# sergivalverde/sub-cortical_segmentation

Hardware: NVIDIA B200
Metric: voxels_per_sec_full_volume_inference (higher is better)
Workload: dtype bf16

## Files before the change

sub-cortical_segmentation_b200/csrc/conv_sweep.cu:

```cuda
#include "tc_common.cuh"

namespace sc {

constexpr int SW_SLOT_HALF = 17408;
constexpr int SW_MAX_SLOTS = 14;
constexpr int SW_BAR_BYTES = 512;

struct SweepArgs {
  int Pw, R;
  int bn;
  int S;
  int nstrips, strip_w;
  int nseg, L;
  int n_items;
  int stages;
  int out_bufs;
  int npanels;
  int in_dx, in_dy;
  const float* scale; const float* shift; const float* alpha;
  unsigned long long* dbg;
  const uint8_t* item_on;
  double* stats;
  int st_H, st_pitch;
};

__device__ __forceinline__ void sweep_mma(uint32_t acc, uint32_t a_lo, uint32_t b_lo, uint32_t idesc, uint32_t accumulate, uint32_t elected) {
  asm volatile(
      "{\n\t"
      ".reg .pred p, q;\n\t"
      ".reg .b64 da, db;\n\t"
      "setp.ne.b32 p, %4, 0;\n\t"
      "setp.ne.b32 q, %5, 0;\n\t"
      "mov.b64 da, {%1, %6};\n\t"
      "mov.b64 db, {%2, %6};\n\t"
      "@q tcgen05.mma.cta_group::1.kind::f16 [%0], da, db, %3, p;\n\t"
      "}" ::"r"(acc), "r"(a_lo), "r"(b_lo), "r"(idesc), "r"(accumulate), "r"(elected), "r"(0x40004040u) : "memory");
}
__device__ __forceinline__ uint32_t desc_lo(uint32_t saddr) { return ((saddr & 0x3FFFFu) >> 4) | (1u << 16); }

__device__ __forceinline__ void tmem_ld16(uint32_t taddr, uint32_t (&r)[16]) {
  asm volatile(
      "tcgen05.ld.sync.aligned.32x32b.x16.b32 {%0, %1, %2, %3, %4, %5, %6, %7, %8, %9, %10, %11, %12, %13, %14, %15}, [%16];"
      : "=r"(r[0]), "=r"(r[1]), "=r"(r[2]), "=r"(r[3]), "=r"(r[4]), "=r"(r[5]), "=r"(r[6]), "=r"(r[7]), "=r"(r[8]),
        "=r"(r[9]), "=r"(r[10]), "=r"(r[11]), "=r"(r[12]), "=r"(r[13]), "=r"(r[14]), "=r"(r[15])
      : "r"(taddr));
}

__device__ __forceinline__ void tmem_ld8(uint32_t taddr, uint32_t (&r)[8]) {
  asm volatile("tcgen05.ld.sync.aligned.32x32b.x8.b32 {%0, %1, %2, %3, %4, %5, %6, %7}, [%8];"
               : "=r"(r[0]), "=r"(r[1]), "=r"(r[2]), "=r"(r[3]), "=r"(r[4]), "=r"(r[5]), "=r"(r[6]), "=r"(r[7])
               : "r"(taddr));
}
template <int CW>
__device__ __forceinline__ void sweep_stats_flush(float (&st_s)[CW], float (&st_q)[CW], float* s_red , int ew, int c0,
                                                  bool real, int lane, double* stats) {
#pragma unroll
  for (int k = 0; k < CW; ++k)
#pragma unroll
    for (int o = 16; o; o >>= 1) { st_s[k] += __shfl_xor_sync(0xffffffffu, st_s[k], o); st_q[k] += __shfl_xor_sync(0xffffffffu, st_q[k], o); }
  if (lane == 0) {
#pragma unroll
    for (int k = 0; k < CW; ++k) { s_red[ew * 2 * CW + k] = st_s[k]; s_red[ew * 2 * CW + CW + k] = st_q[k]; }
  }
  asm volatile("bar.sync 7, 512;" ::: "memory");
  if ((ew & 3) == 0 && real && lane < 2 * CW) {
    const int base = ew * 2 * CW + lane;
    const float tot = s_red[base] + s_red[base + 2 * CW] + s_red[base + 4 * CW] + s_red[base + 6 * CW];
    const int mom = lane / CW, ch = c0 + (lane - mom * CW);
    if (ch < 64) atomicAdd(&stats[ch * 2 + mom], (double)tot);
  }
}

template <int CW>
__device__ __forceinline__ void tmem_ld(uint32_t taddr, uint32_t (&r)[CW]) {
  if constexpr (CW == 16) tmem_ld16(taddr, r); else tmem_ld8(taddr, r);
}
template <int CW>
__device__ __forceinline__ void tmem_zero(uint32_t taddr) {
  if constexpr (CW == 16)
    asm volatile("tcgen05.st.sync.aligned.32x32b.x16.b32 [%0], {%1, %1, %1, %1, %1, %1, %1, %1, %1, %1, %1, %1, %1, %1, %1, %1};"
                 ::"r"(taddr), "r"(0u) : "memory");
  else
    asm volatile("tcgen05.st.sync.aligned.32x32b.x8.b32 [%0], {%1, %1, %1, %1, %1, %1, %1, %1};" ::"r"(taddr), "r"(0u) : "memory");
}
template <int CW>
__device__ __forceinline__ void sweep_acc_clear(uint32_t tcol, int S, int bn) {
  for (int j = 0; j < S + 2; ++j) tmem_zero<CW>(tcol + (uint32_t)(j * bn));
  asm volatile("tcgen05.wait::st.sync.aligned;" ::: "memory");
}
template <int CW, bool PAIR>
__device__ __forceinline__ void sweep_drain(uint64_t* afull, uint64_t* aempty, uint32_t& dj, uint32_t& dph, int S, int bn,
                                            uint32_t tcol, bool real, bool keep, int lane, float (&acc)[CW], bool timed,
                                            uint32_t& w_wait) {
  const long long c0 = timed ? clock64() : 0;
  mbar_wait(&afull[dj], (dph >> dj) & 1u);
  dph ^= 1u << dj;
  if (timed) w_wait += (uint32_t)(clock64() - c0);
  asm volatile("tcgen05.fence::after_thread_sync;" ::: "memory");
  if (real) {
    const uint32_t taddr = tcol + dj * (uint32_t)bn, tspill = taddr + (uint32_t)(S * bn);
    const bool split = dj < 2;
    if (keep) {
#pragma unroll
      for (int h = 0; h < CW; h += 8) {
        uint32_t r1[8], r2[8];
        tmem_ld8(taddr + h, r1);
        if (split) tmem_ld8(tspill + h, r2);
        asm volatile("tcgen05.wait::ld.sync.aligned;" ::: "memory");
#pragma unroll
        for (int k = 0; k < 8; ++k) acc[h + k] = split ? __uint_as_float(r1[k]) + __uint_as_float(r2[k]) : __uint_as_float(r1[k]);
      }
    }
    tmem_zero<CW>(taddr);
    if (split) tmem_zero<CW>(tspill);
    asm volatile("tcgen05.wait::st.sync.aligned;" ::: "memory");
  }
  asm volatile("tcgen05.fence::before_thread_sync;" ::: "memory");
  __syncwarp();
  if (lane == 0) {
    if (PAIR) mbar_arrive_cta(&aempty[dj], 0); else mbar_arrive(&aempty[dj]);
  }
  if (++dj == (uint32_t)S) dj = 0;
}
__device__ __forceinline__ void sweep_claim(uint64_t* aempty, uint32_t j, uint32_t& eph) {
  mbar_wait(&aempty[j], ((eph >> j) & 1u) ^ 1u);
  eph ^= 1u << j;
}
__device__ __forceinline__ uint32_t slot_back(uint32_t j, uint32_t k, int S) { return j >= k ? j - k : j + (uint32_t)S - k; }
__device__ __forceinline__ void tma_store_3d(const CUtensorMap* map, const void* src, int c0, int c1, int c2) {
  asm volatile("cp.async.bulk.tensor.3d.global.shared::cta.bulk_group [%0, {%2, %3, %4}], [%1];"
               ::"l"(reinterpret_cast<uint64_t>(map)), "r"(smem_u32(src)), "r"(c0), "r"(c1), "r"(c2) : "memory");
}
template <int KSTEPS, int DIL, int POOL, int CW, bool LO64, bool OUT32>
__global__ void __launch_bounds__(576, 1)
conv_sweep_kernel(const __grid_constant__ CUtensorMap mapA, const __grid_constant__ CUtensorMap mapW, const __grid_constant__ CUtensorMap mapO,
                  const SweepArgs a) {
  extern __shared__ uint8_t smem_raw[];
  uint8_t* smem = smem_raw + ((1024u - (smem_u32(smem_raw) & 1023u)) & 1023u);
  constexpr int BOXPX = 128 + 2 * DIL;
  constexpr int BOX_BYTES = BOXPX * 128;
  constexpr int NBOX = LO64 ? 1 : 2;
  constexpr int SLOT = NBOX * SW_SLOT_HALF;
  constexpr int LO_OFF = LO64 ? 64 : SW_SLOT_HALF;
  const int half_bytes = 3 * a.bn * 128;
  const int panel_bytes = 2 * half_bytes;
  const int w_bytes = a.npanels * panel_bytes;
  uint8_t* sW = smem;
  uint8_t* sRing = smem + w_bytes;
  constexpr int OB_BYTES = OUT32 ? 16384 : 32768;
  uint8_t* sOut = sRing + a.stages * SLOT;
  uint64_t* bars = reinterpret_cast<uint64_t*>(sOut + a.out_bufs * OB_BYTES);
  uint64_t* full = bars;
  uint64_t* empty = bars + a.stages;
  uint64_t* afull = bars + 2 * a.stages;
  uint64_t* aempty = afull + a.S;
  uint64_t* wfull = aempty + a.S;
  uint32_t* tmem_slot = reinterpret_cast<uint32_t*>(wfull + 1);
  float* s_const = reinterpret_cast<float*>(tmem_slot + 2);
  float* s_xch = s_const + 192;

  const int warp = threadIdx.x >> 5, lane = threadIdx.x & 31;

  if (threadIdx.x == 0) {
    for (int s = 0; s < a.stages; ++s) { mbar_init(&full[s], 1); mbar_init(&empty[s], 1); }
    for (int j = 0; j < a.S; ++j) { mbar_init(&afull[j], 1); mbar_init(&aempty[j], 16); }
    mbar_init(wfull, 1);
    asm volatile("fence.mbarrier_init.release.cluster;" ::: "memory");
  }
  if (warp == 1) {
    asm volatile("tcgen05.alloc.cta_group::1.sync.aligned.shared::cta.b32 [%0], %1;" ::"r"(smem_u32(tmem_slot)), "r"(512) : "memory");
    asm volatile("tcgen05.relinquish_alloc_permit.cta_group::1.sync.aligned;" ::: "memory");
  }
  for (int i = threadIdx.x; i < 64; i += blockDim.x) {
    const bool ok = i < a.bn;
    s_const[i] = ok ? __ldg(a.scale + i) : 0.f;
    s_const[64 + i] = ok ? __ldg(a.shift + i) : 0.f;
    s_const[128 + i] = ok ? __ldg(a.alpha + i) : 0.f;
  }
  for (int i = threadIdx.x; i < a.out_bufs * OB_BYTES / 16; i += blockDim.x)
    reinterpret_cast<uint4*>(sOut)[i] = make_uint4(0u, 0u, 0u, 0u);
  asm volatile("fence.proxy.async.shared::cta;" ::: "memory");
  asm volatile("tcgen05.fence::before_thread_sync;" ::: "memory");
  __syncthreads();
  asm volatile("tcgen05.fence::after_thread_sync;" ::: "memory");
  const uint32_t tmem_base = *tmem_slot;
  const int q4 = warp & 3, ew = warp - 2, grp = ew >> 2, c0 = grp * CW;
  const bool real = c0 < a.bn;
  const uint32_t tcol = tmem_base + ((uint32_t)(q4 * 32) << 16) + (uint32_t)c0;
  if (warp >= 2 && real) sweep_acc_clear<CW>(tcol, a.S, a.bn);
  asm volatile("tcgen05.fence::before_thread_sync;" ::: "memory");
  __syncthreads();
  asm volatile("tcgen05.fence::after_thread_sync;" ::: "memory");

  auto decode = [&](int item, int& w0, int& q, int& n0, int& Lc) {
    const int strip = item % a.nstrips;
    const int rest = item / a.nstrips;
    q = rest % DIL;
    const int seg = rest / DIL;
    w0 = strip * a.strip_w;
    const int Nq = (a.R - q + DIL - 1) / DIL;
    n0 = seg * a.L;
    Lc = Nq - n0 < a.L ? Nq - n0 : a.L;
  };

  if (warp == 0) {
    if (lane == 0) {
      asm volatile("prefetch.tensormap [%0];" ::"l"(reinterpret_cast<uint64_t>(&mapA)) : "memory");
      asm volatile("prefetch.tensormap [%0];" ::"l"(reinterpret_cast<uint64_t>(&mapW)) : "memory");
      asm volatile("prefetch.tensormap [%0];" ::"l"(reinterpret_cast<uint64_t>(&mapO)) : "memory");
      mbar_expect_tx(wfull, (uint32_t)w_bytes);
      for (int p = 0; p < 2 * a.npanels; ++p) tma_load_2d(&mapW, wfull, sW + p * half_bytes, 0, p * 3 * a.bn);
      uint32_t g = 0;
      long long w_empty = 0;
      const long long tstart = a.dbg ? clock64() : 0;
      for (int item = blockIdx.x; item < a.n_items; item += gridDim.x) {
        int w0, q, n0, Lc;
        decode(item, w0, q, n0, Lc);
        if (Lc <= 0 || (a.item_on && !a.item_on[item])) continue;
        const int nload = Lc + (POOL == 1 ? 1 : 0) + 2;
        for (int m = 0; m < nload; ++m, ++g) {
          const uint32_t s = g % a.stages, use = g / a.stages;
          if (use > 0) {
            const long long c0 = a.dbg ? clock64() : 0;
            mbar_wait(&empty[s], (use - 1) & 1);
            if (a.dbg) w_empty += clock64() - c0;
          }
          mbar_expect_tx(&full[s], (uint32_t)(NBOX * BOX_BYTES));
          uint8_t* sp = sRing + s * SLOT;
          const int r = q + DIL * (n0 + m);
          tma_load_3d(&mapA, &full[s], sp, 0, w0 + a.in_dx, r + a.in_dy);
          if (NBOX == 2) tma_load_3d(&mapA, &full[s], sp + SW_SLOT_HALF, 64, w0 + a.in_dx, r + a.in_dy);
        }
      }
      if (a.dbg) { a.dbg[blockIdx.x * 8 + 0] = (unsigned long long)w_empty; a.dbg[blockIdx.x * 8 + 1] = (unsigned long long)(clock64() - tstart); }
    }
    __syncwarp();
  } else if (warp == 1) {
    const uint32_t leader = elect_one();
    const uint32_t idesc = (1u << 4) | (1u << 7) | (1u << 10) | ((uint32_t)(3 * a.bn >> 3) << 17) | ((uint32_t)(128 >> 4) << 24);
    mbar_wait(wfull, 0);
    const uint32_t w_lo = desc_lo(smem_u32(sW));
    const uint32_t ring_lo = desc_lo(smem_u32(sRing));
    const uint32_t panel16 = (uint32_t)(panel_bytes >> 4), wl_off = (uint32_t)(half_bytes >> 4);
    uint32_t rs = 0, rph = 0;
    uint32_t j = 2, eph = 0;
    bool open = false;
    long long w_full = 0, w_tempty = 0;
    const long long tstart = a.dbg ? clock64() : 0;
    for (int item = blockIdx.x; item < a.n_items; item += gridDim.x) {
      int w0, q, n0, Lc;
      decode(item, w0, q, n0, Lc);
      if (Lc <= 0 || (a.item_on && !a.item_on[item])) continue;
      const int nin = Lc + (POOL == 1 ? 1 : 0) + 2;
      const uint32_t j0 = (uint32_t)(n0 + 2) % (uint32_t)a.S;
      const uint32_t d = open ? (j0 + (uint32_t)a.S - j) % (uint32_t)a.S : 2u;
      if (d) {
        if (open && leader) { umma_commit(&afull[slot_back(j, 2, a.S)]); if (d >= 2) umma_commit(&afull[slot_back(j, 1, a.S)]); }
        if (d >= 2) sweep_claim(aempty, slot_back(j0, 2, a.S), eph);
        sweep_claim(aempty, slot_back(j0, 1, a.S), eph);
      }
      j = j0; open = true;
      for (int m = 0; m < nin; ++m) {
        long long c0 = a.dbg ? clock64() : 0;
        sweep_claim(aempty, j, eph);
        if (a.dbg) { const long long c1 = clock64(); w_tempty += c1 - c0; c0 = c1; }
        mbar_wait(&full[rs], rph);
        if (a.dbg) w_full += clock64() - c0;
        asm volatile("tcgen05.fence::after_thread_sync;" ::: "memory");
        const uint32_t p = slot_back(j, 2, a.S);
        const uint32_t acc = tmem_base + p * (uint32_t)a.bn;
        const uint32_t sl = ring_lo + rs * (SLOT >> 4);
#pragma unroll
        for (int kx = 0; kx < 3; ++kx) {
#pragma unroll
          for (int ks = 0; ks < KSTEPS; ++ks) {
            const int gk = kx * KSTEPS + ks;
            const uint32_t a_hi = sl + (uint32_t)(kx * DIL * 8 + ks * 2);
            const uint32_t a_lo = a_hi + (uint32_t)(LO_OFF >> 4);
            const uint32_t wh = w_lo + (uint32_t)(gk >> 2) * panel16 + (uint32_t)((gk & 3) * 2);
            sweep_mma(acc, a_lo, wh, idesc, 1, leader);
            sweep_mma(acc, a_hi, wh + wl_off, idesc, 1, leader);
            sweep_mma(acc, a_hi, wh, idesc, 1, leader);
          }
        }
        if (leader) {
          umma_commit(&empty[rs]);
          umma_commit(&afull[p]);
        }
        __syncwarp();
        if (++rs == (uint32_t)a.stages) { rs = 0; rph ^= 1; }
        if (++j == (uint32_t)a.S) j = 0;
      }
    }
    if (open && leader) {
      umma_commit(&afull[slot_back(j, 2, a.S)]);
      umma_commit(&afull[slot_back(j, 1, a.S)]);
    }
    __syncwarp();
    if (a.dbg && leader) {
      a.dbg[blockIdx.x * 8 + 2] = (unsigned long long)w_full; a.dbg[blockIdx.x * 8 + 3] = (unsigned long long)w_tempty;
      a.dbg[blockIdx.x * 8 + 4] = (unsigned long long)(clock64() - tstart);
    }
  } else {
    const int px = q4 * 32 + lane;
    const bool issuer = threadIdx.x == 64;
    const int trow = POOL == 2 ? px >> 1 : px;
    const bool writer = POOL == 2 ? !(lane & 1) : true;
    const uint32_t row_off = (uint32_t)trow * 128u;
    const uint32_t sw = (uint32_t)(trow & 7);
    const uint32_t hi_chunk = (uint32_t)(c0 >> 3);
    const uint32_t lo_base = OUT32 ? 0u : 16384u, lo_chunk = OUT32 ? 4u + hi_chunk : hi_chunk;
    uint32_t t = 0, e = 0;
    uint32_t dj = 0, dph = 0;
    uint32_t w_tfull = 0;
    const bool timed = a.dbg != nullptr;
    const long long tstart = a.dbg ? clock64() : 0;
    constexpr bool STATS = POOL == 0 && DIL == 1;
    float st_s[STATS ? CW : 1], st_q[STATS ? CW : 1];
#pragma unroll
    for (int k = 0; k < (STATS ? CW : 1); ++k) st_s[k] = st_q[k] = 0.f;
    float v[CW];
    for (int item = blockIdx.x; item < a.n_items; item += gridDim.x) {
      int w0, q, n0, Lc;
      decode(item, w0, q, n0, Lc);
      if (Lc <= 0 || (a.item_on && !a.item_on[item])) continue;
      const int nrow = Lc + (POOL == 1 ? 1 : 0);
      const uint32_t j0 = (uint32_t)(n0 + 2) % (uint32_t)a.S;
      const uint32_t d = (j0 + 2u * (uint32_t)a.S - 2u - dj) % (uint32_t)a.S;
      if (t == 0 || d >= 3) {
        if (t > 0)
          for (int h = 0; h < 2; ++h) sweep_drain<CW, false>(afull, aempty, dj, dph, a.S, a.bn, tcol, real, false, lane, v, timed, w_tfull);
        dj = slot_back(j0, 2, a.S);
      } else {
        for (uint32_t h = 0; h < d; ++h) sweep_drain<CW, false>(afull, aempty, dj, dph, a.S, a.bn, tcol, real, false, lane, v, timed, w_tfull);
      }
      for (int h = 0; h < 2; ++h) sweep_drain<CW, false>(afull, aempty, dj, dph, a.S, a.bn, tcol, real, false, lane, v, timed, w_tfull);
      float hprev[CW];
#pragma unroll
      for (int k = 0; k < CW; ++k) hprev[k] = 0.f;
      for (int m = 0; m < nrow; ++m, ++t) {
        sweep_drain<CW, false>(afull, aempty, dj, dph, a.S, a.bn, tcol, real, true, lane, v, timed, w_tfull);
        if (real) {
#pragma unroll
          for (int k4 = 0; k4 < CW / 4; ++k4) {
            const float4 sc_ = *reinterpret_cast<const float4*>(s_const + c0 + 4 * k4);
            const float4 sh = *reinterpret_cast<const float4*>(s_const + 64 + c0 + 4 * k4);
            const float4 al = *reinterpret_cast<const float4*>(s_const + 128 + c0 + 4 * k4);
            v[4 * k4 + 0] = prelu(fmaf(v[4 * k4 + 0], sc_.x, sh.x), al.x);
            v[4 * k4 + 1] = prelu(fmaf(v[4 * k4 + 1], sc_.y, sh.y), al.y);
            v[4 * k4 + 2] = prelu(fmaf(v[4 * k4 + 2], sc_.z, sh.z), al.z);
            v[4 * k4 + 3] = prelu(fmaf(v[4 * k4 + 3], sc_.w, sh.w), al.w);
          }
        }

        int r_out = q + DIL * (n0 + m);
        if (POOL == 1) {
          if (real) {
            float* xw = s_xch + (((t & 1) * 4 + grp) * 4 + q4) * 32;
            if (lane < DIL) {
#pragma unroll
              for (int k4 = 0; k4 < CW / 4; ++k4)
                *reinterpret_cast<float4*>(xw + lane * 16 + 4 * k4) = make_float4(v[4 * k4], v[4 * k4 + 1], v[4 * k4 + 2], v[4 * k4 + 3]);
            }
            asm volatile("bar.sync %0, 128;" ::"r"(1 + grp) : "memory");
            const bool edge = lane >= 32 - DIL;
            const float* xr = s_xch + (((t & 1) * 4 + grp) * 4 + ((q4 + 1) & 3)) * 32 + (edge ? (lane - (32 - DIL)) * 16 : 0);
#pragma unroll
            for (int k4 = 0; k4 < CW / 4; ++k4) {
              const float4 x4 = *reinterpret_cast<const float4*>(xr + 4 * k4);
              const float xs[4] = {x4.x, x4.y, x4.z, x4.w};
#pragma unroll
              for (int k = 0; k < 4; ++k) {
                float nb = __shfl_down_sync(0xffffffffu, v[4 * k4 + k], DIL);
                if (edge) nb = xs[k];
                const float h = fmaxf(v[4 * k4 + k], nb);
                v[4 * k4 + k] = fmaxf(h, hprev[4 * k4 + k]);
                hprev[4 * k4 + k] = h;
              }
            }
          }
          if (m == 0) continue;
          r_out -= DIL;
        }
        if (POOL == 2) {
          if (real) {
#pragma unroll
            for (int k = 0; k < CW; ++k) {
              const float h = fmaxf(v[k], __shfl_down_sync(0xffffffffu, v[k], 1));
              v[k] = fmaxf(h, hprev[k]);
              hprev[k] = (m & 1) ? 0.f : h;
            }
          }
          if (!(m & 1)) continue;
          r_out >>= 1;
        }
        if constexpr (STATS) {
          if (a.stats && real) {
            const int wpx = w0 + px;
            if (wpx < a.Pw && (wpx & (a.st_pitch - 1)) < a.st_H && r_out < a.st_H) {
#pragma unroll
              for (int k = 0; k < CW; ++k) { st_s[k] += v[k]; st_q[k] = fmaf(v[k], v[k], st_q[k]); }
            }
          }
        }
        uint8_t* ob = sOut + (e % (uint32_t)a.out_bufs) * OB_BYTES;
        if (a.out_bufs == 1) {
          if (issuer) asm volatile("cp.async.bulk.wait_group.read 0;" ::: "memory");
          asm volatile("bar.sync 5, 512;" ::: "memory");
        }
        if (real) {
          uint32_t hi[CW / 2], lo[CW / 2];
#pragma unroll
          for (int k = 0; k < CW / 2; ++k) split2(v[2 * k], v[2 * k + 1], hi[k], lo[k]);
#pragma unroll
          for (int c = 0; c < CW / 8; ++c) {
            if (!writer) break;
            *reinterpret_cast<uint4*>(ob + row_off + (((hi_chunk + c) ^ sw) << 4)) = make_uint4(hi[4 * c], hi[4 * c + 1], hi[4 * c + 2], hi[4 * c + 3]);
            *reinterpret_cast<uint4*>(ob + lo_base + row_off + (((lo_chunk + c) ^ sw) << 4)) = make_uint4(lo[4 * c], lo[4 * c + 1], lo[4 * c + 2], lo[4 * c + 3]);
          }
          asm volatile("fence.proxy.async.shared::cta;" ::: "memory");
        }
        if (a.out_bufs == 2 && issuer) asm volatile("cp.async.bulk.wait_group.read 0;" ::: "memory");
        asm volatile("bar.sync 6, 512;" ::: "memory");
        if (issuer) {
          tma_store_3d(&mapO, ob, 0, POOL == 2 ? w0 >> 1 : w0, r_out);
          if (!OUT32) tma_store_3d(&mapO, ob + 16384, 64, POOL == 2 ? w0 >> 1 : w0, r_out);
          asm volatile("cp.async.bulk.commit_group;" ::: "memory");
        }
        ++e;
      }
    }
    if (t > 0)
      for (int h = 0; h < 2; ++h) sweep_drain<CW, false>(afull, aempty, dj, dph, a.S, a.bn, tcol, real, false, lane, v, timed, w_tfull);
    if (issuer) asm volatile("cp.async.bulk.wait_group 0;" ::: "memory");
    if constexpr (STATS) {
      if (a.stats) sweep_stats_flush<CW>(st_s, st_q, s_xch, ew, c0, real, lane, a.stats);
    }
    if (a.dbg && threadIdx.x == 64) {
      a.dbg[blockIdx.x * 8 + 5] = (unsigned long long)w_tfull; a.dbg[blockIdx.x * 8 + 6] = (unsigned long long)(clock64() - tstart);
      a.dbg[blockIdx.x * 8 + 7] = t;
    }
  }
  asm volatile("tcgen05.fence::before_thread_sync;" ::: "memory");
  __syncthreads();
  if (warp == 1) {
    asm volatile("tcgen05.fence::after_thread_sync;" ::: "memory");
    asm volatile("tcgen05.dealloc.cta_group::1.sync.aligned.b32 %0, %1;" ::"r"(tmem_base), "r"(512) : "memory");
  }
}

__device__ __forceinline__ void sweep_mma_2sm(uint32_t acc, uint32_t a_lo, uint32_t b_lo, uint32_t idesc, uint32_t accumulate, uint32_t elected) {
  asm volatile(
      "{\n\t"
      ".reg .pred p, q;\n\t"
      ".reg .b64 da, db;\n\t"
      "setp.ne.b32 p, %4, 0;\n\t"
      "setp.ne.b32 q, %5, 0;\n\t"
      "mov.b64 da, {%1, %6};\n\t"
      "mov.b64 db, {%2, %6};\n\t"
      "@q tcgen05.mma.cta_group::2.kind::f16 [%0], da, db, %3, p;\n\t"
      "}" ::"r"(acc), "r"(a_lo), "r"(b_lo), "r"(idesc), "r"(accumulate), "r"(elected), "r"(0x40004040u) : "memory");
}

template <int KSTEPS, int DIL, int POOL>
__global__ void __cluster_dims__(2, 1, 1) __launch_bounds__(576, 1)
conv_sweep_pair_kernel(const __grid_constant__ CUtensorMap mapA, const __grid_constant__ CUtensorMap mapW, const __grid_constant__ CUtensorMap mapO,
                       const SweepArgs a) {
  extern __shared__ uint8_t smem_raw[];
  uint8_t* smem = smem_raw + ((1024u - (smem_u32(smem_raw) & 1023u)) & 1023u);
  constexpr int BOXPX = 128 + 2 * DIL;
  constexpr int BOX_BYTES = BOXPX * 128;
  constexpr int SLOT = 2 * SW_SLOT_HALF;
  constexpr int CW = 16;
  const int panel_bytes = 3 * a.bn * 128;
  const int w_bytes = a.npanels * panel_bytes;
  uint8_t* sW = smem;
  uint8_t* sRing = smem + ((w_bytes + 1023) & ~1023);
  constexpr int OB_BYTES = 32768;
  uint8_t* sOut = sRing + a.stages * SLOT;
  uint64_t* bars = reinterpret_cast<uint64_t*>(sOut + a.out_bufs * OB_BYTES);
  uint64_t* full = bars;
  uint64_t* empty = bars + a.stages;
  uint64_t* afull = bars + 2 * a.stages;
  uint64_t* aempty = afull + a.S;
  uint64_t* wfull = aempty + a.S;
  uint32_t* tmem_slot = reinterpret_cast<uint32_t*>(wfull + 1);
  float* s_const = reinterpret_cast<float*>(tmem_slot + 2);
  float* s_xch = s_const + 192;

  const int warp = threadIdx.x >> 5, lane = threadIdx.x & 31;
  const uint32_t rank = cluster_ctarank();
  const int pair = blockIdx.x >> 1, npairs = gridDim.x >> 1;

  if (threadIdx.x == 0) {
    for (int s = 0; s < a.stages; ++s) { mbar_init(&full[s], 1); mbar_init(&empty[s], 1); }
    for (int j = 0; j < a.S; ++j) { mbar_init(&afull[j], 1); mbar_init(&aempty[j], 32); }
    mbar_init(wfull, 1);
    asm volatile("fence.mbarrier_init.release.cluster;" ::: "memory");
  }
  if (warp == 1) {
    asm volatile("tcgen05.alloc.cta_group::2.sync.aligned.shared::cta.b32 [%0], %1;" ::"r"(smem_u32(tmem_slot)), "r"(512) : "memory");
    asm volatile("tcgen05.relinquish_alloc_permit.cta_group::2.sync.aligned;" ::: "memory");
  }
  for (int i = threadIdx.x; i < 64; i += blockDim.x) {
    const bool ok = i < a.bn;
    s_const[i] = ok ? __ldg(a.scale + i) : 0.f;
    s_const[64 + i] = ok ? __ldg(a.shift + i) : 0.f;
    s_const[128 + i] = ok ? __ldg(a.alpha + i) : 0.f;
  }
  for (int i = threadIdx.x; i < a.out_bufs * OB_BYTES / 16; i += blockDim.x)
    reinterpret_cast<uint4*>(sOut)[i] = make_uint4(0u, 0u, 0u, 0u);
  asm volatile("fence.proxy.async.shared::cta;" ::: "memory");
  asm volatile("tcgen05.fence::before_thread_sync;" ::: "memory");
  __syncthreads();
  asm volatile("tcgen05.fence::after_thread_sync;" ::: "memory");
  const uint32_t tmem_base = *tmem_slot;
  const int q4 = warp & 3, ew = warp - 2, grp = ew >> 2, c0 = grp * CW;
  const bool real = c0 < a.bn;
  const uint32_t tcol = tmem_base + ((uint32_t)(q4 * 32) << 16) + (uint32_t)c0;
  if (warp >= 2 && real) sweep_acc_clear<CW>(tcol, a.S, a.bn);
  asm volatile("tcgen05.fence::before_thread_sync;" ::: "memory");
  __syncthreads();
  cluster_sync_all();
  asm volatile("tcgen05.fence::after_thread_sync;" ::: "memory");

  const int nsp = (a.nstrips + 1) >> 1;
  auto decode = [&](int item, int& w0, int& q, int& n0, int& Lc) {
    const int sp = item % nsp;
    const int rest = item / nsp;
    q = rest % DIL;
    const int seg = rest / DIL;
    w0 = (2 * sp + (int)rank) * a.strip_w;
    const int Nq = (a.R - q + DIL - 1) / DIL;
    n0 = seg * a.L;
    Lc = Nq - n0 < a.L ? Nq - n0 : a.L;
  };

  if (warp == 0) {
    if (lane == 0) {
      asm volatile("prefetch.tensormap [%0];" ::"l"(reinterpret_cast<uint64_t>(&mapA)) : "memory");
      asm volatile("prefetch.tensormap [%0];" ::"l"(reinterpret_cast<uint64_t>(&mapW)) : "memory");
      asm volatile("prefetch.tensormap [%0];" ::"l"(reinterpret_cast<uint64_t>(&mapO)) : "memory");
      {
        const uint32_t lbar = smem_u32(wfull) & 0xFEFFFFFFu;
        if (rank == 0) mbar_expect_tx(wfull, (uint32_t)(2 * w_bytes));
        for (int p = 0; p < a.npanels; ++p) tma_load_2d_2sm(&mapW, lbar, sW + p * panel_bytes, 0, (p * 2 + (int)rank) * 3 * a.bn);
      }
      uint32_t g = 0;
      long long w_empty = 0;
      const long long tstart = a.dbg ? clock64() : 0;
      for (int item = pair; item < a.n_items; item += npairs) {
        int w0, q, n0, Lc;
        decode(item, w0, q, n0, Lc);
        if (Lc <= 0 || (a.item_on && !a.item_on[item])) continue;
        const int nload = Lc + (POOL == 1 ? 1 : 0) + 2;
        for (int m = 0; m < nload; ++m, ++g) {
          const uint32_t s = g % a.stages, use = g / a.stages;
          if (use > 0) {
            const long long c0w = a.dbg ? clock64() : 0;
            mbar_wait(&empty[s], (use - 1) & 1);
            if (a.dbg) w_empty += clock64() - c0w;
          }
          const uint32_t lbar = smem_u32(&full[s]) & 0xFEFFFFFFu;
          if (rank == 0) mbar_expect_tx(&full[s], (uint32_t)(2 * 2 * BOX_BYTES));
          uint8_t* sp = sRing + s * SLOT;
          const int r = q + DIL * (n0 + m);
          tma_load_3d_2sm(&mapA, lbar, sp, 0, w0 + a.in_dx, r + a.in_dy);
          tma_load_3d_2sm(&mapA, lbar, sp + SW_SLOT_HALF, 64, w0 + a.in_dx, r + a.in_dy);
        }
      }
      if (a.dbg) { a.dbg[blockIdx.x * 8 + 0] = (unsigned long long)w_empty; a.dbg[blockIdx.x * 8 + 1] = (unsigned long long)(clock64() - tstart); }
    }
    __syncwarp();
  } else if (warp == 1) {
    if (rank == 0) {
      const uint32_t leader = elect_one();
      const uint32_t idesc = (1u << 4) | (1u << 7) | (1u << 10) | ((uint32_t)(3 * a.bn >> 3) << 17) | ((uint32_t)(256 >> 4) << 24);
      mbar_wait(wfull, 0);
      const uint32_t w_lo = desc_lo(smem_u32(sW));
      const uint32_t ring_lo = desc_lo(smem_u32(sRing));
      const uint32_t panel16 = (uint32_t)(panel_bytes >> 4);
      const uint32_t wl_off = (uint32_t)(3 * a.bn / 2 * 128) >> 4;
      uint32_t rs = 0, rph = 0, j = 2, eph = 0;
      bool open = false;
      long long w_full = 0, w_tempty = 0;
      const long long tstart = a.dbg ? clock64() : 0;
      for (int item = pair; item < a.n_items; item += npairs) {
        int w0, q, n0, Lc;
        decode(item, w0, q, n0, Lc);
        if (Lc <= 0 || (a.item_on && !a.item_on[item])) continue;
        const int nin = Lc + (POOL == 1 ? 1 : 0) + 2;
        const uint32_t j0 = (uint32_t)(n0 + 2) % (uint32_t)a.S;
        const uint32_t d = open ? (j0 + (uint32_t)a.S - j) % (uint32_t)a.S : 2u;
        if (d) {
          if (open && leader) { umma_commit_2sm(&afull[slot_back(j, 2, a.S)]); if (d >= 2) umma_commit_2sm(&afull[slot_back(j, 1, a.S)]); }
          if (d >= 2) sweep_claim(aempty, slot_back(j0, 2, a.S), eph);
          sweep_claim(aempty, slot_back(j0, 1, a.S), eph);
        }
        j = j0; open = true;
        for (int m = 0; m < nin; ++m) {
          long long c0w = a.dbg ? clock64() : 0;
          sweep_claim(aempty, j, eph);
          if (a.dbg) { const long long c1 = clock64(); w_tempty += c1 - c0w; c0w = c1; }
          mbar_wait(&full[rs], rph);
          if (a.dbg) w_full += clock64() - c0w;
          asm volatile("tcgen05.fence::after_thread_sync;" ::: "memory");
          const uint32_t p = slot_back(j, 2, a.S);
          const uint32_t acc = tmem_base + p * (uint32_t)a.bn;
          const uint32_t sl = ring_lo + rs * (SLOT >> 4);
#pragma unroll
          for (int kx = 0; kx < 3; ++kx) {
#pragma unroll
            for (int ks = 0; ks < KSTEPS; ++ks) {
              const int gk = kx * KSTEPS + ks;
              const uint32_t a_hi = sl + (uint32_t)(kx * DIL * 8 + ks * 2);
              const uint32_t a_lo = a_hi + (uint32_t)(SW_SLOT_HALF >> 4);
              const uint32_t wh = w_lo + (uint32_t)(gk >> 2) * panel16 + (uint32_t)((gk & 3) * 2);
              sweep_mma_2sm(acc, a_lo, wh, idesc, 1, leader);
              sweep_mma_2sm(acc, a_hi, wh + wl_off, idesc, 1, leader);
              sweep_mma_2sm(acc, a_hi, wh, idesc, 1, leader);
            }
          }
          if (leader) {
            umma_commit_2sm(&empty[rs]);
            umma_commit_2sm(&afull[p]);
          }
          __syncwarp();
          if (++rs == (uint32_t)a.stages) { rs = 0; rph ^= 1; }
          if (++j == (uint32_t)a.S) j = 0;
        }
      }
      if (open && leader) {
        umma_commit_2sm(&afull[slot_back(j, 2, a.S)]);
        umma_commit_2sm(&afull[slot_back(j, 1, a.S)]);
      }
      __syncwarp();
      if (a.dbg && leader) {
        a.dbg[blockIdx.x * 8 + 2] = (unsigned long long)w_full; a.dbg[blockIdx.x * 8 + 3] = (unsigned long long)w_tempty;
        a.dbg[blockIdx.x * 8 + 4] = (unsigned long long)(clock64() - tstart);
      }
    }
  } else {
    const int px = q4 * 32 + lane;
    const bool issuer = threadIdx.x == 64;
    const int trow = POOL == 2 ? px >> 1 : px;
    const bool writer = POOL == 2 ? !(lane & 1) : true;
    const uint32_t row_off = (uint32_t)trow * 128u;
    const uint32_t sw = (uint32_t)(trow & 7);
    const uint32_t hi_chunk = (uint32_t)(c0 >> 3);
    uint32_t t = 0, e = 0, dj = 0, dph = 0;
    uint32_t w_tfull = 0;
    const bool timed = a.dbg != nullptr;
    const long long tstart = a.dbg ? clock64() : 0;
    constexpr bool STATS = POOL == 0 && DIL == 1;
    float st_s[STATS ? CW : 1], st_q[STATS ? CW : 1];
#pragma unroll
    for (int k = 0; k < (STATS ? CW : 1); ++k) st_s[k] = st_q[k] = 0.f;
    float v[CW];
    for (int item = pair; item < a.n_items; item += npairs) {
      int w0, q, n0, Lc;
      decode(item, w0, q, n0, Lc);
      if (Lc <= 0 || (a.item_on && !a.item_on[item])) continue;
      const int nrow = Lc + (POOL == 1 ? 1 : 0);
      const uint32_t j0 = (uint32_t)(n0 + 2) % (uint32_t)a.S;
      const uint32_t d = (j0 + 2u * (uint32_t)a.S - 2u - dj) % (uint32_t)a.S;
      if (t == 0 || d >= 3) {
        if (t > 0)
          for (int h = 0; h < 2; ++h) sweep_drain<CW, true>(afull, aempty, dj, dph, a.S, a.bn, tcol, real, false, lane, v, timed, w_tfull);
        dj = slot_back(j0, 2, a.S);
      } else {
        for (uint32_t h = 0; h < d; ++h) sweep_drain<CW, true>(afull, aempty, dj, dph, a.S, a.bn, tcol, real, false, lane, v, timed, w_tfull);
      }
      for (int h = 0; h < 2; ++h) sweep_drain<CW, true>(afull, aempty, dj, dph, a.S, a.bn, tcol, real, false, lane, v, timed, w_tfull);
      float hprev[CW];
#pragma unroll
      for (int k = 0; k < CW; ++k) hprev[k] = 0.f;
      for (int m = 0; m < nrow; ++m, ++t) {
        sweep_drain<CW, true>(afull, aempty, dj, dph, a.S, a.bn, tcol, real, true, lane, v, timed, w_tfull);
        if (real) {
#pragma unroll
          for (int k4 = 0; k4 < CW / 4; ++k4) {
            const float4 sc_ = *reinterpret_cast<const float4*>(s_const + c0 + 4 * k4);
            const float4 sh = *reinterpret_cast<const float4*>(s_const + 64 + c0 + 4 * k4);
            const float4 al = *reinterpret_cast<const float4*>(s_const + 128 + c0 + 4 * k4);
            v[4 * k4 + 0] = prelu(fmaf(v[4 * k4 + 0], sc_.x, sh.x), al.x);
            v[4 * k4 + 1] = prelu(fmaf(v[4 * k4 + 1], sc_.y, sh.y), al.y);
            v[4 * k4 + 2] = prelu(fmaf(v[4 * k4 + 2], sc_.z, sh.z), al.z);
            v[4 * k4 + 3] = prelu(fmaf(v[4 * k4 + 3], sc_.w, sh.w), al.w);
          }
        }

        int r_out = q + DIL * (n0 + m);
        if (POOL == 1) {
          if (real) {
            float* xw = s_xch + (((t & 1) * 4 + grp) * 4 + q4) * 32;
            if (lane < DIL) {
#pragma unroll
              for (int k4 = 0; k4 < CW / 4; ++k4)
                *reinterpret_cast<float4*>(xw + lane * 16 + 4 * k4) = make_float4(v[4 * k4], v[4 * k4 + 1], v[4 * k4 + 2], v[4 * k4 + 3]);
            }
            asm volatile("bar.sync %0, 128;" ::"r"(1 + grp) : "memory");
            const bool edge = lane >= 32 - DIL;
            const float* xr = s_xch + (((t & 1) * 4 + grp) * 4 + ((q4 + 1) & 3)) * 32 + (edge ? (lane - (32 - DIL)) * 16 : 0);
#pragma unroll
            for (int k4 = 0; k4 < CW / 4; ++k4) {
              const float4 x4 = *reinterpret_cast<const float4*>(xr + 4 * k4);
              const float xs[4] = {x4.x, x4.y, x4.z, x4.w};
#pragma unroll
              for (int k = 0; k < 4; ++k) {
                float nb = __shfl_down_sync(0xffffffffu, v[4 * k4 + k], DIL);
                if (edge) nb = xs[k];
                const float h = fmaxf(v[4 * k4 + k], nb);
                v[4 * k4 + k] = fmaxf(h, hprev[4 * k4 + k]);
                hprev[4 * k4 + k] = h;
              }
            }
          }
          if (m == 0) continue;
          r_out -= DIL;
        }
        if (POOL == 2) {
          if (real) {
#pragma unroll
            for (int k = 0; k < CW; ++k) {
              const float h = fmaxf(v[k], __shfl_down_sync(0xffffffffu, v[k], 1));
              v[k] = fmaxf(h, hprev[k]);
              hprev[k] = (m & 1) ? 0.f : h;
            }
          }
          if (!(m & 1)) continue;
          r_out >>= 1;
        }
        if constexpr (STATS) {
          if (a.stats && real) {
            const int wpx = w0 + px;
            if (wpx < a.Pw && (wpx & (a.st_pitch - 1)) < a.st_H && r_out < a.st_H) {
#pragma unroll
              for (int k = 0; k < CW; ++k) { st_s[k] += v[k]; st_q[k] = fmaf(v[k], v[k], st_q[k]); }
            }
          }
        }
        uint8_t* ob = sOut + (e % (uint32_t)a.out_bufs) * OB_BYTES;
        if (a.out_bufs == 1) {
          if (issuer) asm volatile("cp.async.bulk.wait_group.read 0;" ::: "memory");
          asm volatile("bar.sync 5, 512;" ::: "memory");
        }
        if (real) {
          uint32_t hi[CW / 2], lo[CW / 2];
#pragma unroll
          for (int k = 0; k < CW / 2; ++k) split2(v[2 * k], v[2 * k + 1], hi[k], lo[k]);
#pragma unroll
          for (int c = 0; c < CW / 8; ++c) {
            if (!writer) break;
            *reinterpret_cast<uint4*>(ob + row_off + (((hi_chunk + c) ^ sw) << 4)) = make_uint4(hi[4 * c], hi[4 * c + 1], hi[4 * c + 2], hi[4 * c + 3]);
            *reinterpret_cast<uint4*>(ob + 16384 + row_off + (((hi_chunk + c) ^ sw) << 4)) = make_uint4(lo[4 * c], lo[4 * c + 1], lo[4 * c + 2], lo[4 * c + 3]);
          }
          asm volatile("fence.proxy.async.shared::cta;" ::: "memory");
        }
        if (a.out_bufs == 2 && issuer) asm volatile("cp.async.bulk.wait_group.read 0;" ::: "memory");
        asm volatile("bar.sync 6, 512;" ::: "memory");
        if (issuer) {
          tma_store_3d(&mapO, ob, 0, POOL == 2 ? w0 >> 1 : w0, r_out);
          tma_store_3d(&mapO, ob + 16384, 64, POOL == 2 ? w0 >> 1 : w0, r_out);
          asm volatile("cp.async.bulk.commit_group;" ::: "memory");
        }
        ++e;
      }
    }
    if (t > 0)
      for (int h = 0; h < 2; ++h) sweep_drain<CW, true>(afull, aempty, dj, dph, a.S, a.bn, tcol, real, false, lane, v, timed, w_tfull);
    if (issuer) asm volatile("cp.async.bulk.wait_group 0;" ::: "memory");
    if constexpr (STATS) {
      if (a.stats) sweep_stats_flush<CW>(st_s, st_q, s_xch, ew, c0, real, lane, a.stats);
    }
    if (a.dbg && threadIdx.x == 64) {
      a.dbg[blockIdx.x * 8 + 5] = (unsigned long long)w_tfull; a.dbg[blockIdx.x * 8 + 6] = (unsigned long long)(clock64() - tstart);
      a.dbg[blockIdx.x * 8 + 7] = t;
    }
  }
  asm volatile("tcgen05.fence::before_thread_sync;" ::: "memory");
  __syncthreads();
  cluster_sync_all();
  if (warp == 1) {
    asm volatile("tcgen05.fence::after_thread_sync;" ::: "memory");
    asm volatile("tcgen05.dealloc.cta_group::2.sync.aligned.b32 %0, %1;" ::"r"(tmem_base), "r"(512) : "memory");
  }
}

__device__ __forceinline__ void tma_store_4d(const CUtensorMap* map, const void* src, int c0, int c1, int c2, int c3) {
  asm volatile("cp.async.bulk.tensor.4d.global.shared::cta.bulk_group [%0, {%2, %3, %4, %5}], [%1];"
               ::"l"(reinterpret_cast<uint64_t>(map)), "r"(smem_u32(src)), "r"(c0), "r"(c1), "r"(c2), "r"(c3) : "memory");
}

__global__ void __launch_bounds__(256) conv1_wide_kernel(const __grid_constant__ CUtensorMap mapO, const __grid_constant__ Conv1Consts cw,
                                                         const float* __restrict__ vol, ViewGeo g, int ns, int outR, int outC, int slice_fast) {
  extern __shared__ uint8_t smem_raw[];
  uint8_t* tiles = smem_raw + ((1024u - (smem_u32(smem_raw) & 1023u)) & 1023u);
  const int bc = slice_fast ? 8 : 32, bs = slice_fast ? 32 : 8;
  const int nct = (outC + bc - 1) / bc, nst = (ns + bs - 1) / bs;
  const long long n_tiles = (long long)outR * nst * nct;
  const int f = threadIdx.x & 31, sl = threadIdx.x >> 5;
  const int cl = slice_fast ? sl : f, sloc = slice_fast ? f : sl;
  const int trow = sloc * bc + cl;
  const uint32_t row_off = (uint32_t)trow * 128u, swz = (uint32_t)(trow & 7);
  uint32_t it = 0;
  for (long long t = blockIdx.x; t < n_tiles; t += gridDim.x, ++it) {
    const int ct = (int)(t % nct);
    const int stl = (int)((t / nct) % nst);
    const int i = (int)(t / ((long long)nct * nst));
    const int j = ct * bc + cl, s = stl * bs + sloc;
    uint8_t* ob = tiles + (it & 1) * 32768;
    if (it >= 2) {
      if (threadIdx.x == 0) asm volatile("cp.async.bulk.wait_group.read 1;" ::: "memory");
      __syncthreads();
    }
    float v[20];
    if (j < outC && s < ns) {
      const float* vb = vol + (int64_t)(g.s0 + s) * g.ss;
      float x[9];
#pragma unroll
      for (int ky = 0; ky < 3; ++ky) {
        const int rr = g.r0 + i + ky - 16;
#pragma unroll
        for (int kx = 0; kx < 3; ++kx) {
          const int cc = g.c0 + j + kx - 16;
          x[ky * 3 + kx] = (rr >= 0 && rr < g.R && cc >= 0 && cc < g.C) ? __ldg(vb + (int64_t)rr * g.rs + (int64_t)cc * g.cs) : 0.f;
        }
      }
#pragma unroll
      for (int co = 0; co < 20; ++co) {
        float acc = 0.f;
#pragma unroll
        for (int tp = 0; tp < 9; ++tp) acc = fmaf(x[tp], cw.w[tp * 20 + co], acc);
        v[co] = prelu(fmaf(acc, cw.scale[co], cw.shift[co]), cw.alpha[co]);
      }
    } else {
#pragma unroll
      for (int co = 0; co < 20; ++co) v[co] = 0.f;
    }
    uint32_t hi[12], lo[12];
#pragma unroll
    for (int k = 0; k < 10; ++k) split2(v[2 * k], v[2 * k + 1], hi[k], lo[k]);
    hi[10] = hi[11] = lo[10] = lo[11] = 0u;
#pragma unroll
    for (int c = 0; c < 3; ++c) {
      *reinterpret_cast<uint4*>(ob + row_off + (((uint32_t)c ^ swz) << 4)) = make_uint4(hi[4 * c], hi[4 * c + 1], hi[4 * c + 2], hi[4 * c + 3]);
      *reinterpret_cast<uint4*>(ob + row_off + (((uint32_t)(4 + c) ^ swz) << 4)) = make_uint4(lo[4 * c], lo[4 * c + 1], lo[4 * c + 2], lo[4 * c + 3]);
    }
    *reinterpret_cast<uint4*>(ob + row_off + ((3u ^ swz) << 4)) = make_uint4(0u, 0u, 0u, 0u);
    *reinterpret_cast<uint4*>(ob + row_off + ((7u ^ swz) << 4)) = make_uint4(0u, 0u, 0u, 0u);
    asm volatile("fence.proxy.async.shared::cta;" ::: "memory");
    __syncthreads();
    if (threadIdx.x == 0) {
      tma_store_4d(&mapO, ob, 0, ct * bc, stl * bs, i);
      asm volatile("cp.async.bulk.commit_group;" ::: "memory");
    }
  }
  if (threadIdx.x == 0) asm volatile("cp.async.bulk.wait_group 0;" ::: "memory");
}

int launch_conv1_wide(sc_ctx* ctx, const float* vol, const ViewGeo& g, int ns, const Conv1Consts& cw, float* out, int outR, int outC,
                      cudaStream_t st) {
  TcState* s = reinterpret_cast<TcState*>(ctx->tc_state);
  SC_CHECK(s != nullptr, SC_ERR_UNSUPPORTED, "tcgen05 back-end not initialised");
  if (ns <= 0 || outR <= 0 || outC <= 0) return SC_OK;
  const int slice_fast = (g.ss == 1 && g.cs != 1) ? 1 : 0;
  const int bc = slice_fast ? 8 : 32, bs = slice_fast ? 32 : 8;
  CUtensorMap mapO;
  cuuint64_t dims[4] = {64, (cuuint64_t)outC, (cuuint64_t)ns, (cuuint64_t)outR};
  cuuint64_t strides[3] = {128, (cuuint64_t)outC * 128, (cuuint64_t)ns * outC * 128};
  cuuint32_t box[4] = {64, (cuuint32_t)bc, (cuuint32_t)bs, 1};
  cuuint32_t es[4] = {1, 1, 1, 1};
  CUresult r = s->encode(&mapO, CU_TENSOR_MAP_DATA_TYPE_BFLOAT16, 4, out, dims, strides, box, es, CU_TENSOR_MAP_INTERLEAVE_NONE,
                         CU_TENSOR_MAP_SWIZZLE_128B, CU_TENSOR_MAP_L2_PROMOTION_NONE, CU_TENSOR_MAP_FLOAT_OOB_FILL_NONE);
  SC_CHECK(r == CUDA_SUCCESS, SC_ERR_CUDA, "conv1_wide: cuTensorMapEncodeTiled failed with %d", (int)r);
  SC_TRY(ensure_smem_attr(ctx, reinterpret_cast<const void*>(conv1_wide_kernel), 2 * 32768 + 1024));
  const long long n_tiles = (long long)outR * ((ns + bs - 1) / bs) * ((outC + bc - 1) / bc);
  const long long cap = (long long)ctx->sm_count * 3;
  const unsigned grid = (unsigned)(n_tiles < cap ? n_tiles : cap);
  ProfScope prof(ctx, PC_CONV1, st);
  conv1_wide_kernel<<<grid, 256, 2 * 32768 + 1024, st>>>(mapO, cw, vol, g, ns, outR, outC, slice_fast);
  ctx->launches++;
  SC_CUDA(cudaGetLastError());
  return SC_OK;
}

template <int KSTEPS, int DIL, int POOL, int CW, bool LO64, bool OUT32>
static int launch_sweep_t(sc_ctx* ctx, const CUtensorMap& mapA, const CUtensorMap& mapW, const CUtensorMap& mapO, const SweepArgs& a,
                          size_t smem, cudaStream_t st) {
  auto kern = conv_sweep_kernel<KSTEPS, DIL, POOL, CW, LO64, OUT32>;
  SC_TRY(ensure_smem_attr(ctx, reinterpret_cast<const void*>(kern), 227 * 1024));
  const int grid = a.n_items < ctx->sm_count ? a.n_items : ctx->sm_count;
  kern<<<grid, 576, smem, st>>>(mapA, mapW, mapO, a);
  ctx->launches++;
  SC_CUDA(cudaGetLastError());
  return SC_OK;
}

__global__ void __launch_bounds__(256) view_occupancy_kernel(const uint8_t* __restrict__ cand, ViewGeo g, uint32_t* __restrict__ occ) {
  const int64_t w = (int64_t)blockIdx.x * 8 + (threadIdx.x >> 5);
  if (w >= (int64_t)g.br * g.ns) return;
  const int lane = threadIdx.x & 31;
  const int i = (int)(w / g.ns), sl = (int)(w - (int64_t)i * g.ns);
  const uint8_t* base = cand + (int64_t)(g.s0 + sl) * g.ss + (int64_t)(g.r0 + i) * g.rs + (int64_t)g.c0 * g.cs;
  uint32_t bits = 0;
  for (int jb = 0; jb * 32 < g.bc; ++jb) {
    const int j = jb * 32 + lane;
    const bool on = j < g.bc && base[(int64_t)j * g.cs] != 0;
    if (__any_sync(0xffffffffu, on)) bits |= 1u << jb;
  }
  if (lane == 0) occ[w] = bits;
}

int launch_view_occupancy(sc_ctx* ctx, const uint8_t* cand, const ViewGeo& g, uint32_t* occ, cudaStream_t st) {
  SC_CHECK(g.bc <= 1024, SC_ERR_ARG, "sweep skip: more than 1024 columns per slice");
  const int64_t warps = (int64_t)g.br * g.ns;
  view_occupancy_kernel<<<(unsigned)((warps + 7) / 8), 256, 0, st>>>(cand, g, occ);
  ctx->launches++;
  SC_CUDA(cudaGetLastError());
  return SC_OK;
}

__global__ void __launch_bounds__(256) sweep_item_flags_kernel(const uint32_t* __restrict__ occ, int br, int bc, int ns, int C1, int reach, int n_items,
                                                               int nstr, int dil, int L, int R, int item_w, int Pw, uint8_t* __restrict__ flags) {
  const int item = blockIdx.x * 8 + (threadIdx.x >> 5);
  if (item >= n_items) return;
  const int lane = threadIdx.x & 31;
  const int strip = item % nstr, rest = item / nstr;
  const int q = rest % dil, seg = rest / dil;
  const int Nq = (R - q + dil - 1) / dil;
  const int n0 = seg * L;
  const int Lc = Nq - n0 < L ? Nq - n0 : L;
  bool any = false;
  if (Lc > 0) {
    const int rlo = q + dil * n0, rhi = q + dil * (n0 + Lc - 1);
    const int ilo = rlo - reach > 0 ? rlo - reach : 0, ihi = rhi < br - 1 ? rhi : br - 1;
    const int w0 = strip * item_w;
    int w1 = w0 + item_w - 1;
    if (w1 > Pw - 1) w1 = Pw - 1;
    if (w0 <= w1 && ilo <= ihi) {
      const int sa = w0 / C1, sb = w1 / C1;
      const int nrow = ihi - ilo + 1;
      for (int e = lane; e < nrow * (sb - sa + 1); e += 32) {
        const int sl = sa + e / nrow, i = ilo + e % nrow;
        if (sl >= ns) continue;
        const int clo = w0 - sl * C1 > 0 ? w0 - sl * C1 : 0;
        const int chi = w1 - sl * C1 < C1 - 1 ? w1 - sl * C1 : C1 - 1;
        const int jlo = clo - reach > 0 ? clo - reach : 0, jhi = chi < bc - 1 ? chi : bc - 1;
        if (jlo > jhi) continue;
        const int b0 = jlo >> 5, b1 = jhi >> 5;
        const uint32_t colmask = (b1 - b0 == 31 ? 0xffffffffu : ((1u << (b1 - b0 + 1)) - 1u)) << b0;
        if (occ[(int64_t)i * ns + sl] & colmask) any = true;
      }
    }
  }
  any = __any_sync(0xffffffffu, any);
  if (lane == 0) flags[item] = any ? 1 : 0;
}

static int launch_item_flags(sc_ctx* ctx, const SweepSkip* skip, SweepArgs& a, int nstr, int item_w, int dil, int rows_out, cudaStream_t st) {
  if (!skip) return SC_OK;
  sweep_item_flags_kernel<<<(unsigned)((a.n_items + 7) / 8), 256, 0, st>>>(skip->occ, skip->br, skip->bc, skip->ns, skip->C1, rows_out - skip->br,
                                                                         a.n_items, nstr, dil, a.L, a.R, item_w, a.Pw, skip->flags);
  ctx->launches++;
  SC_CUDA(cudaGetLastError());
  a.item_on = skip->flags;
  return SC_OK;
}

int launch_conv_sweep(sc_ctx* ctx, const SweepW& w, int layer, const float* in, int in_fmt, float* out, int out_fmt,
                      int Pw, int R, int rows_out, int dil, int pool, int prof_cls, cudaStream_t st, int in_dx, int in_dy, const SweepSkip* skip,
                      const SweepStats* stats) {
  TcState* s = reinterpret_cast<TcState*>(ctx->tc_state);
  SC_CHECK(s != nullptr, SC_ERR_UNSUPPORTED, "tcgen05 back-end not initialised");
  if (Pw <= 0 || R <= 0) return SC_OK;
  SweepArgs a;
  if (rows_out <= 0 || rows_out > R) rows_out = R;
  a.Pw = Pw; a.R = rows_out; a.bn = w.bn;
  a.strip_w = 128 - (pool == 1 ? dil : 0);
  a.nstrips = (Pw + a.strip_w - 1) / a.strip_w;
  const int nq = (rows_out + dil - 1) / dil;
  int nseg = (4 * ctx->sm_count + a.nstrips * dil - 1) / (a.nstrips * dil);
  int L = (nq + nseg - 1) / nseg;
  if (L < 12) L = 12;
  if (a.nstrips * dil * ((nq + 11) / 12) < ctx->sm_count) {
    nseg = (ctx->sm_count + a.nstrips * dil - 1) / (a.nstrips * dil);
    L = (nq + nseg - 1) / nseg;
    if (L < 2) L = 2;
  }
  if (L > 96) L = 96;
  if (skip && L > 32) L = 32;
  if (pool == 2) L = (L + 1) & ~1;
  nseg = (nq + L - 1) / L;
  a.L = L; a.nseg = nseg;
  a.n_items = a.nstrips * dil * nseg;
  a.item_on = nullptr;
  a.stats = nullptr; a.st_H = 0; a.st_pitch = 1;
  if (stats) {
    SC_CHECK(dil == 1 && !pool && (stats->pitch & (stats->pitch - 1)) == 0, SC_ERR_ARG, "conv_sweep: fused statistics need dil 1, no pool, a power-of-two pitch");
    a.stats = stats->sums; a.st_H = stats->H; a.st_pitch = stats->pitch;
  }
  SC_CHECK(pool != 2 || dil == 1, SC_ERR_ARG, "conv_sweep: the stride-2 pool needs dilation 1");
  a.npanels = w.npanels;
  a.in_dx = in_dx; a.in_dy = in_dy;
  a.scale = w.scale; a.shift = w.shift; a.alpha = w.alpha;
  a.dbg = (ctx->tc_timing_cls == prof_cls) ? ctx->tc_timing_buf : nullptr;
  SC_CHECK(w.bn <= (out_fmt ? 32 : 64) && w.bn % 16 == 0, SC_ERR_ARG, "conv_sweep: bad channel geometry");
  a.S = 512 / w.bn - 2;
  if (a.S > SW_MAX_SLOTS) a.S = SW_MAX_SLOTS;
  const int slot = (in_fmt ? 1 : 2) * SW_SLOT_HALF;
  const int w_bytes = w.npanels * 6 * w.bn * 128;
  const int ob_bytes = out_fmt ? 16384 : 32768;
  const int fixed = 1024 + w_bytes + SW_BAR_BYTES + 192 * 4 + 2 * 4 * 4 * 2 * 16 * 4;
  a.out_bufs = 2;
  a.stages = (227 * 1024 - fixed - 2 * ob_bytes) / slot;
  if (a.stages < 3) {
    a.out_bufs = 1;
    a.stages = (227 * 1024 - fixed - ob_bytes) / slot;
  }
  if (a.stages > 8) a.stages = 8;
  const bool use_pair = w.ksteps >= 3 && !in_fmt && !out_fmt;
  SC_CHECK(use_pair || a.stages >= 2, SC_ERR_ARG, "conv_sweep: ring does not fit (layer %d)", layer);
  const size_t smem = (size_t)fixed + (size_t)a.stages * slot + (size_t)a.out_bufs * ob_bytes;

  CUtensorMap mapA, mapW, mapO;
  {
    const int pxe = in_fmt ? 64 : 128;
    cuuint64_t dims[3] = {(cuuint64_t)pxe, (cuuint64_t)Pw, (cuuint64_t)R};
    cuuint64_t strides[2] = {(cuuint64_t)pxe * 2, (cuuint64_t)Pw * pxe * 2};
    cuuint32_t box[3] = {64, (cuuint32_t)(128 + 2 * dil), 1};
    cuuint32_t es[3] = {1, 1, 1};
    CUresult r = s->encode(&mapA, CU_TENSOR_MAP_DATA_TYPE_BFLOAT16, 3, const_cast<float*>(in), dims, strides, box, es,
                           CU_TENSOR_MAP_INTERLEAVE_NONE, CU_TENSOR_MAP_SWIZZLE_128B, CU_TENSOR_MAP_L2_PROMOTION_L2_256B,
                           CU_TENSOR_MAP_FLOAT_OOB_FILL_NONE);
    SC_CHECK(r == CUDA_SUCCESS, SC_ERR_CUDA, "conv_sweep: cuTensorMapEncodeTiled(A) failed with %d (Pw %d R %d)", (int)r, Pw, R);
  }
  {
    cuuint64_t dims[2] = {64, (cuuint64_t)w.npanels * 6 * w.bn};
    cuuint64_t strides[1] = {128};
    cuuint32_t box[2] = {64, (cuuint32_t)(3 * w.bn)};
    cuuint32_t es[2] = {1, 1};
    CUresult r = s->encode(&mapW, CU_TENSOR_MAP_DATA_TYPE_BFLOAT16, 2, w.panels, dims, strides, box, es,
                           CU_TENSOR_MAP_INTERLEAVE_NONE, CU_TENSOR_MAP_SWIZZLE_128B, CU_TENSOR_MAP_L2_PROMOTION_L2_256B,
                           CU_TENSOR_MAP_FLOAT_OOB_FILL_NONE);
    SC_CHECK(r == CUDA_SUCCESS, SC_ERR_CUDA, "conv_sweep: cuTensorMapEncodeTiled(W) failed with %d", (int)r);
  }
  {
    const int pxe = out_fmt ? 64 : 128;
    const int oPw = pool == 2 ? Pw / 2 : Pw, oR = pool == 2 ? R / 2 : R;
    cuuint64_t dims[3] = {(cuuint64_t)pxe, (cuuint64_t)oPw, (cuuint64_t)oR};
    cuuint64_t strides[2] = {(cuuint64_t)pxe * 2, (cuuint64_t)oPw * pxe * 2};
    cuuint32_t box[3] = {64, (cuuint32_t)(pool == 2 ? 64 : a.strip_w), 1};
    cuuint32_t es[3] = {1, 1, 1};
    CUresult r = s->encode(&mapO, CU_TENSOR_MAP_DATA_TYPE_BFLOAT16, 3, out, dims, strides, box, es,
                           CU_TENSOR_MAP_INTERLEAVE_NONE, CU_TENSOR_MAP_SWIZZLE_128B, CU_TENSOR_MAP_L2_PROMOTION_NONE,
                           CU_TENSOR_MAP_FLOAT_OOB_FILL_NONE);
    SC_CHECK(r == CUDA_SUCCESS, SC_ERR_CUDA, "conv_sweep: cuTensorMapEncodeTiled(O) failed with %d", (int)r);
  }
  const bool i32 = in_fmt != 0, o32 = out_fmt != 0;
  if (use_pair) {
    const int nsp = (a.nstrips + 1) / 2;
    const int pairs_max = ctx->sm_count / 2;
    nseg = (4 * pairs_max + nsp * dil - 1) / (nsp * dil);
    L = (nq + nseg - 1) / nseg;
    if (L < 12) L = 12;
    if (nsp * dil * ((nq + 11) / 12) < pairs_max) {
      nseg = (pairs_max + nsp * dil - 1) / (nsp * dil);
      L = (nq + nseg - 1) / nseg;
      if (L < 2) L = 2;
    }
    if (L > 96) L = 96;
    if (skip && L > 32) L = 32;
    if (pool == 2) L = (L + 1) & ~1;
    nseg = (nq + L - 1) / L;
    a.L = L; a.nseg = nseg;
    a.n_items = nsp * dil * nseg;
    const int wp_bytes = w.npanels * 3 * w.bn * 128;
    const int fixed_p = 1024 + ((wp_bytes + 1023) & ~1023) + SW_BAR_BYTES + 192 * 4 + ((pool || stats) ? 2 * 4 * 4 * 2 * 16 * 4 : 0);
    a.out_bufs = 2;
    a.stages = (227 * 1024 - fixed_p - 2 * ob_bytes) / slot;
    if (a.stages < 3) { a.out_bufs = 1; a.stages = (227 * 1024 - fixed_p - ob_bytes) / slot; }
    if (a.stages > 8) a.stages = 8;
    SC_CHECK(a.stages >= 2, SC_ERR_ARG, "conv_sweep: pair ring does not fit (layer %d)", layer);
    SC_CHECK(pool != 2 || (Pw % 2 == 0), SC_ERR_ARG, "conv_sweep: odd pitch with the stride-2 pool");
    const size_t smem_p = (size_t)fixed_p + (size_t)a.stages * slot + (size_t)a.out_bufs * ob_bytes;
    CUtensorMap mapWp;
    cuuint64_t dims[2] = {64, (cuuint64_t)w.npanels * 6 * w.bn};
    cuuint64_t strides[1] = {128};
    cuuint32_t box[2] = {64, (cuuint32_t)(3 * w.bn)};
    cuuint32_t es[2] = {1, 1};
    CUresult r = s->encode(&mapWp, CU_TENSOR_MAP_DATA_TYPE_BFLOAT16, 2, w.panels_pair, dims, strides, box, es,
                           CU_TENSOR_MAP_INTERLEAVE_NONE, CU_TENSOR_MAP_SWIZZLE_128B, CU_TENSOR_MAP_L2_PROMOTION_L2_256B,
                           CU_TENSOR_MAP_FLOAT_OOB_FILL_NONE);
    SC_CHECK(r == CUDA_SUCCESS, SC_ERR_CUDA, "conv_sweep: cuTensorMapEncodeTiled(W pair) failed with %d", (int)r);
    const int npairs = a.n_items < pairs_max ? a.n_items : pairs_max;
    SC_TRY(launch_item_flags(ctx, skip, a, nsp, 2 * a.strip_w, dil, rows_out, st));
    ProfScope prof(ctx, prof_cls, st);
    if (dil == 1 && pool == 2) {
      auto kern = conv_sweep_pair_kernel<3, 1, 2>;
      SC_TRY(ensure_smem_attr(ctx, reinterpret_cast<const void*>(kern), 227 * 1024));
      kern<<<2 * npairs, 576, smem_p, st>>>(mapA, mapWp, mapO, a);
    } else if (dil == 1 && !pool && w.ksteps == 4) {
      auto kern = conv_sweep_pair_kernel<4, 1, 0>;
      SC_TRY(ensure_smem_attr(ctx, reinterpret_cast<const void*>(kern), 227 * 1024));
      kern<<<2 * npairs, 576, smem_p, st>>>(mapA, mapWp, mapO, a);
    } else if (dil == 1 && !pool) {
      auto kern = conv_sweep_pair_kernel<3, 1, 0>;
      SC_TRY(ensure_smem_attr(ctx, reinterpret_cast<const void*>(kern), 227 * 1024));
      kern<<<2 * npairs, 576, smem_p, st>>>(mapA, mapWp, mapO, a);
    } else if (dil == 2 && pool == 1) {
      auto kern = conv_sweep_pair_kernel<3, 2, 1>;
      SC_TRY(ensure_smem_attr(ctx, reinterpret_cast<const void*>(kern), 227 * 1024));
      kern<<<2 * npairs, 576, smem_p, st>>>(mapA, mapWp, mapO, a);
    } else if (dil == 4 && !pool) {
      auto kern = conv_sweep_pair_kernel<3, 4, 0>;
      SC_TRY(ensure_smem_attr(ctx, reinterpret_cast<const void*>(kern), 227 * 1024));
      kern<<<2 * npairs, 576, smem_p, st>>>(mapA, mapWp, mapO, a);
    } else {
      set_error("conv_sweep: no pair kernel instance for dil=%d pool=%d", dil, pool);
      return SC_ERR_ARG;
    }
    ctx->launches++;
    SC_CUDA(cudaGetLastError());
    return SC_OK;
  }
  SC_TRY(launch_item_flags(ctx, skip, a, a.nstrips, a.strip_w, dil, rows_out, st));
  ProfScope prof(ctx, prof_cls, st);
  if (w.ksteps == 2 && dil == 1 && pool == 2 && i32 && o32 && w.bn == 32) return launch_sweep_t<2, 1, 2, 8, true, true>(ctx, mapA, mapW, mapO, a, smem, st);
  if (w.ksteps == 2 && dil == 1 && pool == 1 && i32 && o32 && w.bn == 32) return launch_sweep_t<2, 1, 1, 8, true, true>(ctx, mapA, mapW, mapO, a, smem, st);
  if (w.ksteps == 2 && dil == 2 && !pool && i32 && !o32) return launch_sweep_t<2, 2, 0, 16, true, false>(ctx, mapA, mapW, mapO, a, smem, st);
  if (w.ksteps == 2 && dil == 1 && !pool && i32 && !o32) return launch_sweep_t<2, 1, 0, 16, true, false>(ctx, mapA, mapW, mapO, a, smem, st);
  if (w.ksteps == 2 && dil == 1 && !pool && i32 && o32 && w.bn == 32) return launch_sweep_t<2, 1, 0, 8, true, true>(ctx, mapA, mapW, mapO, a, smem, st);
  set_error("conv_sweep: no kernel instance for ksteps=%d dil=%d pool=%d in_fmt=%d out_fmt=%d", w.ksteps, dil, pool, in_fmt, out_fmt);
  return SC_ERR_ARG;
}

}
```

Measured before the change: 162.7 million.

## Replace block-wide epilogue barriers with per-quarter barriers and split output stores

The epilogue warps stop synchronising all 512 threads before each output row. Each 128-thread quarter now uses its own named barrier and issues its own TMA store slice, with a second tensor map covering the trailing partial quarter. The pool-1 halo exchange moves from a block barrier to per-slot mbarrier handoffs, and the TMEM slot is released right after pooling rather than after the store. This should cut epilogue serialisation and let TMEM slots recycle sooner, at the cost of more barriers and more, smaller TMA stores.

```diff
diff --git a/sub-cortical_segmentation_b200/csrc/conv_sweep.cu b/sub-cortical_segmentation_b200/csrc/conv_sweep.cu
--- a/sub-cortical_segmentation_b200/csrc/conv_sweep.cu
+++ b/sub-cortical_segmentation_b200/csrc/conv_sweep.cu
@@ -5,6 +5,7 @@
 constexpr int SW_SLOT_HALF = 17408;
 constexpr int SW_MAX_SLOTS = 14;
 constexpr int SW_BAR_BYTES = 512;
+constexpr int SW_XCH_FLOATS = 2 * 4 * 3 * 32;
 
 struct SweepArgs {
   int Pw, R;
@@ -88,10 +89,9 @@
   for (int j = 0; j < S + 2; ++j) tmem_zero<CW>(tcol + (uint32_t)(j * bn));
   asm volatile("tcgen05.wait::st.sync.aligned;" ::: "memory");
 }
-template <int CW, bool PAIR>
-__device__ __forceinline__ void sweep_drain(uint64_t* afull, uint64_t* aempty, uint32_t& dj, uint32_t& dph, int S, int bn,
-                                            uint32_t tcol, bool real, bool keep, int lane, float (&acc)[CW], bool timed,
-                                            uint32_t& w_wait) {
+template <int CW>
+__device__ __forceinline__ void sweep_take(uint64_t* afull, uint32_t dj, uint32_t& dph, int S, int bn, uint32_t tcol, bool real, bool keep,
+                                           float (&acc)[CW], bool timed, uint32_t& w_wait) {
   const long long c0 = timed ? clock64() : 0;
   mbar_wait(&afull[dj], (dph >> dj) & 1u);
   dph ^= 1u << dj;
@@ -113,8 +113,11 @@
     }
     tmem_zero<CW>(taddr);
     if (split) tmem_zero<CW>(tspill);
-    asm volatile("tcgen05.wait::st.sync.aligned;" ::: "memory");
-  }
+  }
+}
+template <bool PAIR>
+__device__ __forceinline__ void sweep_give(uint64_t* aempty, uint32_t& dj, int S, bool real, int lane) {
+  if (real) asm volatile("tcgen05.wait::st.sync.aligned;" ::: "memory");
   asm volatile("tcgen05.fence::before_thread_sync;" ::: "memory");
   __syncwarp();
   if (lane == 0) {
@@ -122,19 +125,95 @@
   }
   if (++dj == (uint32_t)S) dj = 0;
 }
+template <int CW, bool PAIR>
+__device__ __forceinline__ void sweep_discard(uint64_t* afull, uint64_t* aempty, uint32_t& dj, uint32_t& dph, int S, int bn, uint32_t tcol,
+                                              bool real, int lane, float (&acc)[CW], bool timed, uint32_t& w_wait) {
+  sweep_take<CW>(afull, dj, dph, S, bn, tcol, real, false, acc, timed, w_wait);
+  sweep_give<PAIR>(aempty, dj, S, real, lane);
+}
+
+template <int CW, int DIL>
+__device__ __forceinline__ void sweep_pool1(float (&v)[CW], float (&hprev)[CW], float* s_xch, uint32_t t, int grp, int q4, int lane) {
+  uint64_t* xfull = reinterpret_cast<uint64_t*>(s_xch + SW_XCH_FLOATS);
+  uint64_t* xempty = xfull + 24;
+  const uint32_t ph = (t >> 1) & 1u;
+  if (q4 > 0 && lane < DIL) {
+    const int x = ((t & 1) * 4 + grp) * 3 + q4 - 1;
+    mbar_wait(&xempty[x], ph ^ 1u);
+    float* xw = s_xch + x * 32 + lane * 16;
+#pragma unroll
+    for (int k4 = 0; k4 < CW / 4; ++k4)
+      *reinterpret_cast<float4*>(xw + 4 * k4) = make_float4(v[4 * k4], v[4 * k4 + 1], v[4 * k4 + 2], v[4 * k4 + 3]);
+    mbar_arrive(&xfull[x]);
+  }
+  const bool edge = q4 < 3 && lane >= 32 - DIL;
+  const int x = ((t & 1) * 4 + grp) * 3 + (q4 < 3 ? q4 : 0);
+  if (edge) mbar_wait(&xfull[x], ph);
+  const float* xr = s_xch + x * 32 + (edge ? (lane - (32 - DIL)) * 16 : 0);
+#pragma unroll
+  for (int k4 = 0; k4 < CW / 4; ++k4) {
+    const float4 x4 = edge ? *reinterpret_cast<const float4*>(xr + 4 * k4) : make_float4(0.f, 0.f, 0.f, 0.f);
+    const float xs[4] = {x4.x, x4.y, x4.z, x4.w};
+#pragma unroll
+    for (int k = 0; k < 4; ++k) {
+      float nb = __shfl_down_sync(0xffffffffu, v[4 * k4 + k], DIL);
+      if (edge) nb = xs[k];
+      const float h = fmaxf(v[4 * k4 + k], nb);
+      v[4 * k4 + k] = fmaxf(h, hprev[4 * k4 + k]);
+      hprev[4 * k4 + k] = h;
+    }
+  }
+  if (edge) mbar_arrive(&xempty[x]);
+}
+
+__device__ __forceinline__ void tma_store_3d(const CUtensorMap* map, const void* src, int c0, int c1, int c2) {
+  asm volatile("cp.async.bulk.tensor.3d.global.shared::cta.bulk_group [%0, {%2, %3, %4}], [%1];"
+               ::"l"(reinterpret_cast<uint64_t>(map)), "r"(smem_u32(src)), "r"(c0), "r"(c1), "r"(c2) : "memory");
+}
+template <int CW, int POOL, bool OUT32>
+__device__ __forceinline__ void sweep_emit(const float (&v)[CW], uint8_t* ob, int out_bufs, bool real, bool writer, bool issuer,
+                                           uint32_t row_off, uint32_t sw, uint32_t hi_chunk, const CUtensorMap* mapO, const CUtensorMap* mapO3,
+                                           int x0, int r_out) {
+  constexpr int QPX = POOL == 2 ? 16 : 32;
+  constexpr uint32_t LO_BASE = OUT32 ? 0u : 16384u, LO_CHUNK = OUT32 ? 4u : 0u;
+  uint32_t tid;
+  asm volatile("mov.u32 %0, %%tid.x;" : "=r"(tid));
+  const int q4 = (int)((tid >> 5) & 3u);
+  if (out_bufs == 1) {
+    if (issuer) asm volatile("cp.async.bulk.wait_group.read 0;" ::: "memory");
+    asm volatile("bar.sync %0, 128;" ::"r"(1 + q4) : "memory");
+  }
+  if (real) {
+    uint32_t hi[CW / 2], lo[CW / 2];
+#pragma unroll
+    for (int k = 0; k < CW / 2; ++k) split2(v[2 * k], v[2 * k + 1], hi[k], lo[k]);
+#pragma unroll
+    for (int c = 0; c < CW / 8; ++c) {
+      if (!writer) break;
+      *reinterpret_cast<uint4*>(ob + row_off + (((hi_chunk + c) ^ sw) << 4)) = make_uint4(hi[4 * c], hi[4 * c + 1], hi[4 * c + 2], hi[4 * c + 3]);
+      *reinterpret_cast<uint4*>(ob + LO_BASE + row_off + (((LO_CHUNK + hi_chunk + c) ^ sw) << 4)) = make_uint4(lo[4 * c], lo[4 * c + 1], lo[4 * c + 2], lo[4 * c + 3]);
+    }
+    asm volatile("fence.proxy.async.shared::cta;" ::: "memory");
+  }
+  if (out_bufs == 2 && issuer) asm volatile("cp.async.bulk.wait_group.read 0;" ::: "memory");
+  asm volatile("bar.sync %0, 128;" ::"r"(1 + q4) : "memory");
+  if (issuer) {
+    const CUtensorMap* m = q4 == 3 ? mapO3 : mapO;
+    const uint32_t qoff = (uint32_t)(q4 * QPX * 128);
+    tma_store_3d(m, ob + qoff, 0, x0 + q4 * QPX, r_out);
+    if (!OUT32) tma_store_3d(m, ob + 16384 + qoff, 64, x0 + q4 * QPX, r_out);
+    asm volatile("cp.async.bulk.commit_group;" ::: "memory");
+  }
+}
 __device__ __forceinline__ void sweep_claim(uint64_t* aempty, uint32_t j, uint32_t& eph) {
   mbar_wait(&aempty[j], ((eph >> j) & 1u) ^ 1u);
   eph ^= 1u << j;
 }
 __device__ __forceinline__ uint32_t slot_back(uint32_t j, uint32_t k, int S) { return j >= k ? j - k : j + (uint32_t)S - k; }
-__device__ __forceinline__ void tma_store_3d(const CUtensorMap* map, const void* src, int c0, int c1, int c2) {
-  asm volatile("cp.async.bulk.tensor.3d.global.shared::cta.bulk_group [%0, {%2, %3, %4}], [%1];"
-               ::"l"(reinterpret_cast<uint64_t>(map)), "r"(smem_u32(src)), "r"(c0), "r"(c1), "r"(c2) : "memory");
-}
 template <int KSTEPS, int DIL, int POOL, int CW, bool LO64, bool OUT32>
 __global__ void __launch_bounds__(576, 1)
 conv_sweep_kernel(const __grid_constant__ CUtensorMap mapA, const __grid_constant__ CUtensorMap mapW, const __grid_constant__ CUtensorMap mapO,
-                  const SweepArgs a) {
+                  const __grid_constant__ CUtensorMap mapO3, const SweepArgs a) {
   extern __shared__ uint8_t smem_raw[];
   uint8_t* smem = smem_raw + ((1024u - (smem_u32(smem_raw) & 1023u)) & 1023u);
   constexpr int BOXPX = 128 + 2 * DIL;
@@ -165,6 +244,8 @@
     for (int s = 0; s < a.stages; ++s) { mbar_init(&full[s], 1); mbar_init(&empty[s], 1); }
     for (int j = 0; j < a.S; ++j) { mbar_init(&afull[j], 1); mbar_init(&aempty[j], 16); }
     mbar_init(wfull, 1);
+    if (POOL == 1)
+      for (int x = 0; x < 48; ++x) mbar_init(reinterpret_cast<uint64_t*>(s_xch + SW_XCH_FLOATS) + x, DIL);
     asm volatile("fence.mbarrier_init.release.cluster;" ::: "memory");
   }
   if (warp == 1) {
@@ -208,6 +289,7 @@
       asm volatile("prefetch.tensormap [%0];" ::"l"(reinterpret_cast<uint64_t>(&mapA)) : "memory");
       asm volatile("prefetch.tensormap [%0];" ::"l"(reinterpret_cast<uint64_t>(&mapW)) : "memory");
       asm volatile("prefetch.tensormap [%0];" ::"l"(reinterpret_cast<uint64_t>(&mapO)) : "memory");
+      asm volatile("prefetch.tensormap [%0];" ::"l"(reinterpret_cast<uint64_t>(&mapO3)) : "memory");
       mbar_expect_tx(wfull, (uint32_t)w_bytes);
       for (int p = 0; p < 2 * a.npanels; ++p) tma_load_2d(&mapW, wfull, sW + p * half_bytes, 0, p * 3 * a.bn);
       uint32_t g = 0;
@@ -303,18 +385,17 @@
     }
   } else {
     const int px = q4 * 32 + lane;
-    const bool issuer = threadIdx.x == 64;
+    const bool issuer = grp == 0 && lane == 0;
     const int trow = POOL == 2 ? px >> 1 : px;
     const bool writer = POOL == 2 ? !(lane & 1) : true;
     const uint32_t row_off = (uint32_t)trow * 128u;
     const uint32_t sw = (uint32_t)(trow & 7);
     const uint32_t hi_chunk = (uint32_t)(c0 >> 3);
-    const uint32_t lo_base = OUT32 ? 0u : 16384u, lo_chunk = OUT32 ? 4u + hi_chunk : hi_chunk;
     uint32_t t = 0, e = 0;
     uint32_t dj = 0, dph = 0;
     uint32_t w_tfull = 0;
     const bool timed = a.dbg != nullptr;
-    const long long tstart = a.dbg ? clock64() : 0;
+    if (timed && threadIdx.x == 64) a.dbg[blockIdx.x * 8 + 6] = (unsigned long long)clock64();
     constexpr bool STATS = POOL == 0 && DIL == 1;
     float st_s[STATS ? CW : 1], st_q[STATS ? CW : 1];
 #pragma unroll
@@ -329,17 +410,17 @@
       const uint32_t d = (j0 + 2u * (uint32_t)a.S - 2u - dj) % (uint32_t)a.S;
       if (t == 0 || d >= 3) {
         if (t > 0)
-          for (int h = 0; h < 2; ++h) sweep_drain<CW, false>(afull, aempty, dj, dph, a.S, a.bn, tcol, real, false, lane, v, timed, w_tfull);
+          for (int h = 0; h < 2; ++h) sweep_discard<CW, false>(afull, aempty, dj, dph, a.S, a.bn, tcol, real, lane, v, timed, w_tfull);
         dj = slot_back(j0, 2, a.S);
       } else {
-        for (uint32_t h = 0; h < d; ++h) sweep_drain<CW, false>(afull, aempty, dj, dph, a.S, a.bn, tcol, real, false, lane, v, timed, w_tfull);
-      }
-      for (int h = 0; h < 2; ++h) sweep_drain<CW, false>(afull, aempty, dj, dph, a.S, a.bn, tcol, real, false, lane, v, timed, w_tfull);
+        for (uint32_t h = 0; h < d; ++h) sweep_discard<CW, false>(afull, aempty, dj, dph, a.S, a.bn, tcol, real, lane, v, timed, w_tfull);
+      }
+      for (int h = 0; h < 2; ++h) sweep_discard<CW, false>(afull, aempty, dj, dph, a.S, a.bn, tcol, real, lane, v, timed, w_tfull);
       float hprev[CW];
 #pragma unroll
       for (int k = 0; k < CW; ++k) hprev[k] = 0.f;
       for (int m = 0; m < nrow; ++m, ++t) {
-        sweep_drain<CW, false>(afull, aempty, dj, dph, a.S, a.bn, tcol, real, true, lane, v, timed, w_tfull);
+        sweep_take<CW>(afull, dj, dph, a.S, a.bn, tcol, real, true, v, timed, w_tfull);
         if (real) {
 #pragma unroll
           for (int k4 = 0; k4 < CW / 4; ++k4) {
@@ -352,45 +433,22 @@
             v[4 * k4 + 3] = prelu(fmaf(v[4 * k4 + 3], sc_.w, sh.w), al.w);
           }
         }
-
+        if (POOL == 1 && real) sweep_pool1<CW, DIL>(v, hprev, s_xch, t, grp, q4, lane);
+        if (POOL == 2 && real) {
+#pragma unroll
+          for (int k = 0; k < CW; ++k) {
+            const float h = fmaxf(v[k], __shfl_down_sync(0xffffffffu, v[k], 1));
+            v[k] = fmaxf(h, hprev[k]);
+            hprev[k] = (m & 1) ? 0.f : h;
+          }
+        }
+        sweep_give<false>(aempty, dj, a.S, real, lane);
         int r_out = q + DIL * (n0 + m);
         if (POOL == 1) {
-          if (real) {
-            float* xw = s_xch + (((t & 1) * 4 + grp) * 4 + q4) * 32;
-            if (lane < DIL) {
-#pragma unroll
-              for (int k4 = 0; k4 < CW / 4; ++k4)
-                *reinterpret_cast<float4*>(xw + lane * 16 + 4 * k4) = make_float4(v[4 * k4], v[4 * k4 + 1], v[4 * k4 + 2], v[4 * k4 + 3]);
-            }
-            asm volatile("bar.sync %0, 128;" ::"r"(1 + grp) : "memory");
-            const bool edge = lane >= 32 - DIL;
-            const float* xr = s_xch + (((t & 1) * 4 + grp) * 4 + ((q4 + 1) & 3)) * 32 + (edge ? (lane - (32 - DIL)) * 16 : 0);
-#pragma unroll
-            for (int k4 = 0; k4 < CW / 4; ++k4) {
-              const float4 x4 = *reinterpret_cast<const float4*>(xr + 4 * k4);
-              const float xs[4] = {x4.x, x4.y, x4.z, x4.w};
-#pragma unroll
-              for (int k = 0; k < 4; ++k) {
-                float nb = __shfl_down_sync(0xffffffffu, v[4 * k4 + k], DIL);
-                if (edge) nb = xs[k];
-                const float h = fmaxf(v[4 * k4 + k], nb);
-                v[4 * k4 + k] = fmaxf(h, hprev[4 * k4 + k]);
-                hprev[4 * k4 + k] = h;
-              }
-            }
-          }
           if (m == 0) continue;
           r_out -= DIL;
         }
         if (POOL == 2) {
-          if (real) {
-#pragma unroll
-            for (int k = 0; k < CW; ++k) {
-              const float h = fmaxf(v[k], __shfl_down_sync(0xffffffffu, v[k], 1));
-              v[k] = fmaxf(h, hprev[k]);
-              hprev[k] = (m & 1) ? 0.f : h;
-            }
-          }
           if (!(m & 1)) continue;
           r_out >>= 1;
         }
@@ -403,41 +461,19 @@
             }
           }
         }
-        uint8_t* ob = sOut + (e % (uint32_t)a.out_bufs) * OB_BYTES;
-        if (a.out_bufs == 1) {
-          if (issuer) asm volatile("cp.async.bulk.wait_group.read 0;" ::: "memory");
-          asm volatile("bar.sync 5, 512;" ::: "memory");
-        }
-        if (real) {
-          uint32_t hi[CW / 2], lo[CW / 2];
-#pragma unroll
-          for (int k = 0; k < CW / 2; ++k) split2(v[2 * k], v[2 * k + 1], hi[k], lo[k]);
-#pragma unroll
-          for (int c = 0; c < CW / 8; ++c) {
-            if (!writer) break;
-            *reinterpret_cast<uint4*>(ob + row_off + (((hi_chunk + c) ^ sw) << 4)) = make_uint4(hi[4 * c], hi[4 * c + 1], hi[4 * c + 2], hi[4 * c + 3]);
-            *reinterpret_cast<uint4*>(ob + lo_base + row_off + (((lo_chunk + c) ^ sw) << 4)) = make_uint4(lo[4 * c], lo[4 * c + 1], lo[4 * c + 2], lo[4 * c + 3]);
-          }
-          asm volatile("fence.proxy.async.shared::cta;" ::: "memory");
-        }
-        if (a.out_bufs == 2 && issuer) asm volatile("cp.async.bulk.wait_group.read 0;" ::: "memory");
-        asm volatile("bar.sync 6, 512;" ::: "memory");
-        if (issuer) {
-          tma_store_3d(&mapO, ob, 0, POOL == 2 ? w0 >> 1 : w0, r_out);
-          if (!OUT32) tma_store_3d(&mapO, ob + 16384, 64, POOL == 2 ? w0 >> 1 : w0, r_out);
-          asm volatile("cp.async.bulk.commit_group;" ::: "memory");
-        }
+        sweep_emit<CW, POOL, OUT32>(v, sOut + (a.out_bufs == 2 ? (e & 1u) * OB_BYTES : 0u), a.out_bufs, real, writer, issuer, row_off, sw,
+                                    hi_chunk, &mapO, &mapO3, POOL == 2 ? w0 >> 1 : w0, r_out);
         ++e;
       }
     }
     if (t > 0)
-      for (int h = 0; h < 2; ++h) sweep_drain<CW, false>(afull, aempty, dj, dph, a.S, a.bn, tcol, real, false, lane, v, timed, w_tfull);
+      for (int h = 0; h < 2; ++h) sweep_discard<CW, false>(afull, aempty, dj, dph, a.S, a.bn, tcol, real, lane, v, timed, w_tfull);
     if (issuer) asm volatile("cp.async.bulk.wait_group 0;" ::: "memory");
     if constexpr (STATS) {
       if (a.stats) sweep_stats_flush<CW>(st_s, st_q, s_xch, ew, c0, real, lane, a.stats);
     }
     if (a.dbg && threadIdx.x == 64) {
-      a.dbg[blockIdx.x * 8 + 5] = (unsigned long long)w_tfull; a.dbg[blockIdx.x * 8 + 6] = (unsigned long long)(clock64() - tstart);
+      a.dbg[blockIdx.x * 8 + 5] = (unsigned long long)w_tfull; a.dbg[blockIdx.x * 8 + 6] = (unsigned long long)clock64() - a.dbg[blockIdx.x * 8 + 6];
       a.dbg[blockIdx.x * 8 + 7] = t;
     }
   }
@@ -465,7 +501,7 @@
 template <int KSTEPS, int DIL, int POOL>
 __global__ void __cluster_dims__(2, 1, 1) __launch_bounds__(576, 1)
 conv_sweep_pair_kernel(const __grid_constant__ CUtensorMap mapA, const __grid_constant__ CUtensorMap mapW, const __grid_constant__ CUtensorMap mapO,
-                       const SweepArgs a) {
+                       const __grid_constant__ CUtensorMap mapO3, const SweepArgs a) {
   extern __shared__ uint8_t smem_raw[];
   uint8_t* smem = smem_raw + ((1024u - (smem_u32(smem_raw) & 1023u)) & 1023u);
   constexpr int BOXPX = 128 + 2 * DIL;
@@ -496,6 +532,8 @@
     for (int s = 0; s < a.stages; ++s) { mbar_init(&full[s], 1); mbar_init(&empty[s], 1); }
     for (int j = 0; j < a.S; ++j) { mbar_init(&afull[j], 1); mbar_init(&aempty[j], 32); }
     mbar_init(wfull, 1);
+    if (POOL == 1)
+      for (int x = 0; x < 48; ++x) mbar_init(reinterpret_cast<uint64_t*>(s_xch + SW_XCH_FLOATS) + x, DIL);
     asm volatile("fence.mbarrier_init.release.cluster;" ::: "memory");
   }
   if (warp == 1) {
@@ -541,6 +579,7 @@
       asm volatile("prefetch.tensormap [%0];" ::"l"(reinterpret_cast<uint64_t>(&mapA)) : "memory");
       asm volatile("prefetch.tensormap [%0];" ::"l"(reinterpret_cast<uint64_t>(&mapW)) : "memory");
       asm volatile("prefetch.tensormap [%0];" ::"l"(reinterpret_cast<uint64_t>(&mapO)) : "memory");
+      asm volatile("prefetch.tensormap [%0];" ::"l"(reinterpret_cast<uint64_t>(&mapO3)) : "memory");
       {
         const uint32_t lbar = smem_u32(wfull) & 0xFEFFFFFFu;
         if (rank == 0) mbar_expect_tx(wfull, (uint32_t)(2 * w_bytes));
@@ -642,7 +681,7 @@
     }
   } else {
     const int px = q4 * 32 + lane;
-    const bool issuer = threadIdx.x == 64;
+    const bool issuer = grp == 0 && lane == 0;
     const int trow = POOL == 2 ? px >> 1 : px;
     const bool writer = POOL == 2 ? !(lane & 1) : true;
     const uint32_t row_off = (uint32_t)trow * 128u;
@@ -651,7 +690,7 @@
     uint32_t t = 0, e = 0, dj = 0, dph = 0;
     uint32_t w_tfull = 0;
     const bool timed = a.dbg != nullptr;
-    const long long tstart = a.dbg ? clock64() : 0;
+    if (timed && threadIdx.x == 64) a.dbg[blockIdx.x * 8 + 6] = (unsigned long long)clock64();
     constexpr bool STATS = POOL == 0 && DIL == 1;
     float st_s[STATS ? CW : 1], st_q[STATS ? CW : 1];
 #pragma unroll
@@ -666,17 +705,17 @@
       const uint32_t d = (j0 + 2u * (uint32_t)a.S - 2u - dj) % (uint32_t)a.S;
       if (t == 0 || d >= 3) {
         if (t > 0)
-          for (int h = 0; h < 2; ++h) sweep_drain<CW, true>(afull, aempty, dj, dph, a.S, a.bn, tcol, real, false, lane, v, timed, w_tfull);
+          for (int h = 0; h < 2; ++h) sweep_discard<CW, true>(afull, aempty, dj, dph, a.S, a.bn, tcol, real, lane, v, timed, w_tfull);
         dj = slot_back(j0, 2, a.S);
       } else {
-        for (uint32_t h = 0; h < d; ++h) sweep_drain<CW, true>(afull, aempty, dj, dph, a.S, a.bn, tcol, real, false, lane, v, timed, w_tfull);
-      }
-      for (int h = 0; h < 2; ++h) sweep_drain<CW, true>(afull, aempty, dj, dph, a.S, a.bn, tcol, real, false, lane, v, timed, w_tfull);
+        for (uint32_t h = 0; h < d; ++h) sweep_discard<CW, true>(afull, aempty, dj, dph, a.S, a.bn, tcol, real, lane, v, timed, w_tfull);
+      }
+      for (int h = 0; h < 2; ++h) sweep_discard<CW, true>(afull, aempty, dj, dph, a.S, a.bn, tcol, real, lane, v, timed, w_tfull);
       float hprev[CW];
 #pragma unroll
       for (int k = 0; k < CW; ++k) hprev[k] = 0.f;
       for (int m = 0; m < nrow; ++m, ++t) {
-        sweep_drain<CW, true>(afull, aempty, dj, dph, a.S, a.bn, tcol, real, true, lane, v, timed, w_tfull);
+        sweep_take<CW>(afull, dj, dph, a.S, a.bn, tcol, real, true, v, timed, w_tfull);
         if (real) {
 #pragma unroll
           for (int k4 = 0; k4 < CW / 4; ++k4) {
@@ -689,45 +728,22 @@
             v[4 * k4 + 3] = prelu(fmaf(v[4 * k4 + 3], sc_.w, sh.w), al.w);
           }
         }
-
+        if (POOL == 1 && real) sweep_pool1<CW, DIL>(v, hprev, s_xch, t, grp, q4, lane);
+        if (POOL == 2 && real) {
+#pragma unroll
+          for (int k = 0; k < CW; ++k) {
+            const float h = fmaxf(v[k], __shfl_down_sync(0xffffffffu, v[k], 1));
+            v[k] = fmaxf(h, hprev[k]);
+            hprev[k] = (m & 1) ? 0.f : h;
+          }
+        }
+        sweep_give<true>(aempty, dj, a.S, real, lane);
         int r_out = q + DIL * (n0 + m);
         if (POOL == 1) {
-          if (real) {
-            float* xw = s_xch + (((t & 1) * 4 + grp) * 4 + q4) * 32;
-            if (lane < DIL) {
-#pragma unroll
-              for (int k4 = 0; k4 < CW / 4; ++k4)
-                *reinterpret_cast<float4*>(xw + lane * 16 + 4 * k4) = make_float4(v[4 * k4], v[4 * k4 + 1], v[4 * k4 + 2], v[4 * k4 + 3]);
-            }
-            asm volatile("bar.sync %0, 128;" ::"r"(1 + grp) : "memory");
-            const bool edge = lane >= 32 - DIL;
-            const float* xr = s_xch + (((t & 1) * 4 + grp) * 4 + ((q4 + 1) & 3)) * 32 + (edge ? (lane - (32 - DIL)) * 16 : 0);
-#pragma unroll
-            for (int k4 = 0; k4 < CW / 4; ++k4) {
-              const float4 x4 = *reinterpret_cast<const float4*>(xr + 4 * k4);
-              const float xs[4] = {x4.x, x4.y, x4.z, x4.w};
-#pragma unroll
-              for (int k = 0; k < 4; ++k) {
-                float nb = __shfl_down_sync(0xffffffffu, v[4 * k4 + k], DIL);
-                if (edge) nb = xs[k];
-                const float h = fmaxf(v[4 * k4 + k], nb);
-                v[4 * k4 + k] = fmaxf(h, hprev[4 * k4 + k]);
-                hprev[4 * k4 + k] = h;
-              }
-            }
-          }
           if (m == 0) continue;
           r_out -= DIL;
         }
         if (POOL == 2) {
-          if (real) {
-#pragma unroll
-            for (int k = 0; k < CW; ++k) {
-              const float h = fmaxf(v[k], __shfl_down_sync(0xffffffffu, v[k], 1));
-              v[k] = fmaxf(h, hprev[k]);
-              hprev[k] = (m & 1) ? 0.f : h;
-            }
-          }
           if (!(m & 1)) continue;
           r_out >>= 1;
         }
@@ -740,41 +756,19 @@
             }
           }
         }
-        uint8_t* ob = sOut + (e % (uint32_t)a.out_bufs) * OB_BYTES;
-        if (a.out_bufs == 1) {
-          if (issuer) asm volatile("cp.async.bulk.wait_group.read 0;" ::: "memory");
-          asm volatile("bar.sync 5, 512;" ::: "memory");
-        }
-        if (real) {
-          uint32_t hi[CW / 2], lo[CW / 2];
-#pragma unroll
-          for (int k = 0; k < CW / 2; ++k) split2(v[2 * k], v[2 * k + 1], hi[k], lo[k]);
-#pragma unroll
-          for (int c = 0; c < CW / 8; ++c) {
-            if (!writer) break;
-            *reinterpret_cast<uint4*>(ob + row_off + (((hi_chunk + c) ^ sw) << 4)) = make_uint4(hi[4 * c], hi[4 * c + 1], hi[4 * c + 2], hi[4 * c + 3]);
-            *reinterpret_cast<uint4*>(ob + 16384 + row_off + (((hi_chunk + c) ^ sw) << 4)) = make_uint4(lo[4 * c], lo[4 * c + 1], lo[4 * c + 2], lo[4 * c + 3]);
-          }
-          asm volatile("fence.proxy.async.shared::cta;" ::: "memory");
-        }
-        if (a.out_bufs == 2 && issuer) asm volatile("cp.async.bulk.wait_group.read 0;" ::: "memory");
-        asm volatile("bar.sync 6, 512;" ::: "memory");
-        if (issuer) {
-          tma_store_3d(&mapO, ob, 0, POOL == 2 ? w0 >> 1 : w0, r_out);
-          tma_store_3d(&mapO, ob + 16384, 64, POOL == 2 ? w0 >> 1 : w0, r_out);
-          asm volatile("cp.async.bulk.commit_group;" ::: "memory");
-        }
+        sweep_emit<CW, POOL, false>(v, sOut + (a.out_bufs == 2 ? (e & 1u) * OB_BYTES : 0u), a.out_bufs, real, writer, issuer, row_off, sw,
+                                    hi_chunk, &mapO, &mapO3, POOL == 2 ? w0 >> 1 : w0, r_out);
         ++e;
       }
     }
     if (t > 0)
-      for (int h = 0; h < 2; ++h) sweep_drain<CW, true>(afull, aempty, dj, dph, a.S, a.bn, tcol, real, false, lane, v, timed, w_tfull);
+      for (int h = 0; h < 2; ++h) sweep_discard<CW, true>(afull, aempty, dj, dph, a.S, a.bn, tcol, real, lane, v, timed, w_tfull);
     if (issuer) asm volatile("cp.async.bulk.wait_group 0;" ::: "memory");
     if constexpr (STATS) {
       if (a.stats) sweep_stats_flush<CW>(st_s, st_q, s_xch, ew, c0, real, lane, a.stats);
     }
     if (a.dbg && threadIdx.x == 64) {
-      a.dbg[blockIdx.x * 8 + 5] = (unsigned long long)w_tfull; a.dbg[blockIdx.x * 8 + 6] = (unsigned long long)(clock64() - tstart);
+      a.dbg[blockIdx.x * 8 + 5] = (unsigned long long)w_tfull; a.dbg[blockIdx.x * 8 + 6] = (unsigned long long)clock64() - a.dbg[blockIdx.x * 8 + 6];
       a.dbg[blockIdx.x * 8 + 7] = t;
     }
   }
@@ -886,12 +880,12 @@
 }
 
 template <int KSTEPS, int DIL, int POOL, int CW, bool LO64, bool OUT32>
-static int launch_sweep_t(sc_ctx* ctx, const CUtensorMap& mapA, const CUtensorMap& mapW, const CUtensorMap& mapO, const SweepArgs& a,
-                          size_t smem, cudaStream_t st) {
+static int launch_sweep_t(sc_ctx* ctx, const CUtensorMap& mapA, const CUtensorMap& mapW, const CUtensorMap& mapO, const CUtensorMap& mapO3,
+                          const SweepArgs& a, size_t smem, cudaStream_t st) {
   auto kern = conv_sweep_kernel<KSTEPS, DIL, POOL, CW, LO64, OUT32>;
   SC_TRY(ensure_smem_attr(ctx, reinterpret_cast<const void*>(kern), 227 * 1024));
   const int grid = a.n_items < ctx->sm_count ? a.n_items : ctx->sm_count;
-  kern<<<grid, 576, smem, st>>>(mapA, mapW, mapO, a);
+  kern<<<grid, 576, smem, st>>>(mapA, mapW, mapO, mapO3, a);
   ctx->launches++;
   SC_CUDA(cudaGetLastError());
   return SC_OK;
@@ -1023,7 +1017,7 @@
   SC_CHECK(use_pair || a.stages >= 2, SC_ERR_ARG, "conv_sweep: ring does not fit (layer %d)", layer);
   const size_t smem = (size_t)fixed + (size_t)a.stages * slot + (size_t)a.out_bufs * ob_bytes;
 
-  CUtensorMap mapA, mapW, mapO;
+  CUtensorMap mapA, mapW, mapO, mapO3;
   {
     const int pxe = in_fmt ? 64 : 128;
     cuuint64_t dims[3] = {(cuuint64_t)pxe, (cuuint64_t)Pw, (cuuint64_t)R};
@@ -1045,14 +1039,15 @@
                            CU_TENSOR_MAP_FLOAT_OOB_FILL_NONE);
     SC_CHECK(r == CUDA_SUCCESS, SC_ERR_CUDA, "conv_sweep: cuTensorMapEncodeTiled(W) failed with %d", (int)r);
   }
-  {
+  const int qpx = pool == 2 ? 16 : 32;
+  for (int k = 0; k < 2; ++k) {
     const int pxe = out_fmt ? 64 : 128;
     const int oPw = pool == 2 ? Pw / 2 : Pw, oR = pool == 2 ? R / 2 : R;
     cuuint64_t dims[3] = {(cuuint64_t)pxe, (cuuint64_t)oPw, (cuuint64_t)oR};
     cuuint64_t strides[2] = {(cuuint64_t)pxe * 2, (cuuint64_t)oPw * pxe * 2};
-    cuuint32_t box[3] = {64, (cuuint32_t)(pool == 2 ? 64 : a.strip_w), 1};
+    cuuint32_t box[3] = {64, (cuuint32_t)(k ? qpx - (128 - a.strip_w) : qpx), 1};
     cuuint32_t es[3] = {1, 1, 1};
-    CUresult r = s->encode(&mapO, CU_TENSOR_MAP_DATA_TYPE_BFLOAT16, 3, out, dims, strides, box, es,
+    CUresult r = s->encode(k ? &mapO3 : &mapO, CU_TENSOR_MAP_DATA_TYPE_BFLOAT16, 3, out, dims, strides, box, es,
                            CU_TENSOR_MAP_INTERLEAVE_NONE, CU_TENSOR_MAP_SWIZZLE_128B, CU_TENSOR_MAP_L2_PROMOTION_NONE,
                            CU_TENSOR_MAP_FLOAT_OOB_FILL_NONE);
     SC_CHECK(r == CUDA_SUCCESS, SC_ERR_CUDA, "conv_sweep: cuTensorMapEncodeTiled(O) failed with %d", (int)r);
@@ -1099,23 +1094,23 @@
     if (dil == 1 && pool == 2) {
       auto kern = conv_sweep_pair_kernel<3, 1, 2>;
       SC_TRY(ensure_smem_attr(ctx, reinterpret_cast<const void*>(kern), 227 * 1024));
-      kern<<<2 * npairs, 576, smem_p, st>>>(mapA, mapWp, mapO, a);
+      kern<<<2 * npairs, 576, smem_p, st>>>(mapA, mapWp, mapO, mapO3, a);
     } else if (dil == 1 && !pool && w.ksteps == 4) {
       auto kern = conv_sweep_pair_kernel<4, 1, 0>;
       SC_TRY(ensure_smem_attr(ctx, reinterpret_cast<const void*>(kern), 227 * 1024));
-      kern<<<2 * npairs, 576, smem_p, st>>>(mapA, mapWp, mapO, a);
+      kern<<<2 * npairs, 576, smem_p, st>>>(mapA, mapWp, mapO, mapO3, a);
     } else if (dil == 1 && !pool) {
       auto kern = conv_sweep_pair_kernel<3, 1, 0>;
       SC_TRY(ensure_smem_attr(ctx, reinterpret_cast<const void*>(kern), 227 * 1024));
-      kern<<<2 * npairs, 576, smem_p, st>>>(mapA, mapWp, mapO, a);
+      kern<<<2 * npairs, 576, smem_p, st>>>(mapA, mapWp, mapO, mapO3, a);
     } else if (dil == 2 && pool == 1) {
       auto kern = conv_sweep_pair_kernel<3, 2, 1>;
       SC_TRY(ensure_smem_attr(ctx, reinterpret_cast<const void*>(kern), 227 * 1024));
-      kern<<<2 * npairs, 576, smem_p, st>>>(mapA, mapWp, mapO, a);
+      kern<<<2 * npairs, 576, smem_p, st>>>(mapA, mapWp, mapO, mapO3, a);
     } else if (dil == 4 && !pool) {
       auto kern = conv_sweep_pair_kernel<3, 4, 0>;
       SC_TRY(ensure_smem_attr(ctx, reinterpret_cast<const void*>(kern), 227 * 1024));
-      kern<<<2 * npairs, 576, smem_p, st>>>(mapA, mapWp, mapO, a);
+      kern<<<2 * npairs, 576, smem_p, st>>>(mapA, mapWp, mapO, mapO3, a);
     } else {
       set_error("conv_sweep: no pair kernel instance for dil=%d pool=%d", dil, pool);
       return SC_ERR_ARG;
@@ -1126,11 +1121,11 @@
   }
   SC_TRY(launch_item_flags(ctx, skip, a, a.nstrips, a.strip_w, dil, rows_out, st));
   ProfScope prof(ctx, prof_cls, st);
-  if (w.ksteps == 2 && dil == 1 && pool == 2 && i32 && o32 && w.bn == 32) return launch_sweep_t<2, 1, 2, 8, true, true>(ctx, mapA, mapW, mapO, a, smem, st);
-  if (w.ksteps == 2 && dil == 1 && pool == 1 && i32 && o32 && w.bn == 32) return launch_sweep_t<2, 1, 1, 8, true, true>(ctx, mapA, mapW, mapO, a, smem, st);
-  if (w.ksteps == 2 && dil == 2 && !pool && i32 && !o32) return launch_sweep_t<2, 2, 0, 16, true, false>(ctx, mapA, mapW, mapO, a, smem, st);
-  if (w.ksteps == 2 && dil == 1 && !pool && i32 && !o32) return launch_sweep_t<2, 1, 0, 16, true, false>(ctx, mapA, mapW, mapO, a, smem, st);
-  if (w.ksteps == 2 && dil == 1 && !pool && i32 && o32 && w.bn == 32) return launch_sweep_t<2, 1, 0, 8, true, true>(ctx, mapA, mapW, mapO, a, smem, st);
+  if (w.ksteps == 2 && dil == 1 && pool == 2 && i32 && o32 && w.bn == 32) return launch_sweep_t<2, 1, 2, 8, true, true>(ctx, mapA, mapW, mapO, mapO3, a, smem, st);
+  if (w.ksteps == 2 && dil == 1 && pool == 1 && i32 && o32 && w.bn == 32) return launch_sweep_t<2, 1, 1, 8, true, true>(ctx, mapA, mapW, mapO, mapO3, a, smem, st);
+  if (w.ksteps == 2 && dil == 2 && !pool && i32 && !o32) return launch_sweep_t<2, 2, 0, 16, true, false>(ctx, mapA, mapW, mapO, mapO3, a, smem, st);
+  if (w.ksteps == 2 && dil == 1 && !pool && i32 && !o32) return launch_sweep_t<2, 1, 0, 16, true, false>(ctx, mapA, mapW, mapO, mapO3, a, smem, st);
+  if (w.ksteps == 2 && dil == 1 && !pool && i32 && o32 && w.bn == 32) return launch_sweep_t<2, 1, 0, 8, true, true>(ctx, mapA, mapW, mapO, mapO3, a, smem, st);
   set_error("conv_sweep: no kernel instance for ksteps=%d dil=%d pool=%d in_fmt=%d out_fmt=%d", w.ksteps, dil, pool, in_fmt, out_fmt);
   return SC_ERR_ARG;
 }
```

After: 164.4 million (median of 6 runs). No clear change (+1.1%).
